# CraigIDent/SpliSER

Measured on AMD Instinct MI355X. Metric: splice sites/sec (+ reads/sec) processed, higher is better.
Workload: dtype int32/u32 counters, f64 SSE

## Files before the change

spliser_amd/csrc/spl_capi.cpp:

```cpp
#include <hip/hip_runtime_api.h>
#include <hip/hip_vector_types.h>

#include <sys/mman.h>

#include <algorithm>
#include <atomic>
#include <unistd.h>
#include <cstdarg>
#include <cstdio>
#include <cstring>
#include <new>
#include <string>
#include <chrono>
#include <condition_variable>
#include <functional>
#include <memory>
#include <mutex>
#include <thread>
#include <vector>

#include "../../include/spliser.h"
#include "spl_bam.h"
#include "spl_inflate.h"
#include "spl_sort.h"
// ... 208 lines not shown
}

extern "C" int spl_prof_enable(int on)
{
    std::lock_guard<std::mutex> lock(splprof::mu());
    for (const splprof::Rec &r : splprof::recs()) { splprof::pool().push_back({r.device, r.a}); splprof::pool().push_back({r.device, r.b}); }
    splprof::recs().clear();
    splprof::g_on.store(on ? 1 : 0);
    return SPL_OK;
}

extern "C" int spl_prof_report(char *buf, int cap)
{
    std::vector<splprof::Rec> recs;
    { std::lock_guard<std::mutex> lock(splprof::mu()); recs = splprof::recs(); }
    int cur = 0;
    const bool have = hipGetDevice(&cur) == hipSuccess;
    struct Sum { std::string name; int calls; double ms, bytes; };
    std::vector<Sum> sums;
    for (const splprof::Rec &r : recs) {
        (void)hipSetDevice(r.device);
        float ms = 0;
        if (hipEventSynchronize(r.b) != hipSuccess || hipEventElapsedTime(&ms, r.a, r.b) != hipSuccess) { (void)hipGetLastError(); continue; }
        size_t k = 0;
        while (k < sums.size() && sums[k].name != r.name) ++k;
        if (k == sums.size()) sums.push_back(Sum{r.name, 0, 0, 0});
        sums[k].calls++; sums[k].ms += ms; sums[k].bytes += r.bytes;
    }
    if (have) (void)hipSetDevice(cur);
    std::sort(sums.begin(), sums.end(), [](const Sum &a, const Sum &b) { return a.ms > b.ms; });
    std::string out = "[";
    for (size_t k = 0; k < sums.size(); ++k) {
        char line[256];
        snprintf(line, sizeof line, "%s{\"kernel\": \"%s\", \"calls\": %d, \"ms\": %.4f, \"bytes\": %.0f}", k ? ", " : "", sums[k].name.c_str(), sums[k].calls, sums[k].ms, sums[k].bytes);
        out += line;
    }
    out += "]";
    if (buf && cap > 0) { strncpy(buf, out.c_str(), (size_t)cap - 1); buf[cap - 1] = 0; }
    return (int)out.size() + 1;
}

struct spl_ctx {
    int device = -1;
    hipStream_t stream = nullptr;
    bool own_stream = false;
    hipEvent_t ev0 = nullptr, ev1 = nullptr;
    hipStream_t tail = nullptr;
    hipEvent_t ev_range[4] = {nullptr, nullptr, nullptr, nullptr}, ev_tail[4] = {nullptr, nullptr, nullptr, nullptr};
    uint64_t n_pass = 0;
    bool tail_pending = false;
    int32_t *d_err = nullptr;
    struct Stage { char *host = nullptr; size_t bytes = 0; hipEvent_t done = nullptr; bool busy = false, locked = false; };
    size_t stage_mb = 32;
    std::vector<Stage> stage;
    size_t stage_next = 0;
    hipStream_t copy = nullptr;
    hipEvent_t ev_copy = nullptr;
    int pack_threads = 1;
    bool stage_timing = false;
    hipEvent_t ev_t0 = nullptr, ev_t1 = nullptr;
    double tm_plan_s = 0, tm_emit_s = 0, tm_copy_ms = 0;
    size_t tm_bytes = 0, tm_pieces = 0;
    int last_grid = 0, last_lds = 0;
    struct Junction { int32_t left, right; uint8_t strand; uint32_t count, anchor_left, anchor_right; };
    std::vector<Junction> junctions;
    float junction_ms = -1.0f;
    int64_t junction_table_bytes = 0;
    std::vector<hipEvent_t> k_ev;
    int k_used = 0;
    bool k_on = false;
    std::vector<hipEvent_t> l_ev;
    int l_used = 0;
};

struct spl_dsites {
    int64_t n_sites = 0, n_part = 0, n_comp = 0;
    char *slab = nullptr;
    size_t slab_bytes = 0;
    int32_t *pos = nullptr;
    uint8_t *strand = nullptr, *flags = nullptr;
    uint4 *meta = nullptr;
    uint32_t *part_off = nullptr;
    int32_t *part_pos = nullptr, *part_site = nullptr, *comp_pos = nullptr;
    int64_t *alpha = nullptr, *edge_cnt = nullptr;
    uint32_t *bucket = nullptr;
    uint32_t n_buckets = 0;
    int32_t bucket_base = 0, bucket_shift = 0;
    bool has_sse_inputs = false;
    int32_t *diff = nullptr;
    int32_t *block_sums = nullptr;
    int32_t diff_stride = 0, scan_blocks = 0;
    int32_t n_dpos = 0;
    int32_t *dpos_first_row = nullptr;
    spl_dbk *dbucket = nullptr;
    uint32_t n_dbuckets = 0;
    int32_t dbase = 0;
    int32_t *flag_pos = nullptr;
    uint4 *jhash = nullptr;
    uint32_t jhash_mask = 0;
    uint4 *jrivals = nullptr;
    uint32_t *beta1 = nullptr, *beta2s = nullptr, *dbl = nullptr;
    size_t counter_bytes = 0;
    uint32_t *queue_n = nullptr;
    int32_t *err = nullptr;
    char *region[3] = {nullptr, nullptr, nullptr};
    size_t off_b2 = 0, off_dbl = 0, off_diff = 0, off_ctl = 0;
    bool region_clean[3] = {false, false, false};
    int cur = 2;
    void point_at(int k)
    {
        cur = k;
        beta1 = (uint32_t *)region[k]; beta2s = (uint32_t *)(region[k] + off_b2); dbl = (uint32_t *)(region[k] + off_dbl);
        diff = (int32_t *)(region[k] + off_diff); queue_n = (uint32_t *)(region[k] + off_ctl);
        err = (int32_t *)(region[k] + off_ctl + 4 * 8 * SPL_COUNTER_STRIDE);
    }
    int64_t *b2_simple = nullptr, *b2_cryptic = nullptr;
    double *b2_weighted = nullptr, *sse = nullptr;
    double *sse_cryptic = nullptr;
    bool sse_fused = false;
    const double *sse_view = nullptr;
};

struct DeviceReads;
struct spl_dreads {
    struct Segment {
        char *slab = nullptr;
        uint64_t rec_bytes = 0, n_wide = 0;
        int64_t n_reads = 0, n_ops = 0;
        int32_t shift = 0;
        std::vector<splpack::ChunkDesc> chunks;
        int group = -1;
        size_t group_seg = 0;
    };
    struct Group {
        DeviceReads *src = nullptr;
        std::vector<spl_layout_seg> segs;
        uint32_t n_chunks = 0;
        char *slab = nullptr;
        spl_layout_seg *d_segs = nullptr;
        spl_layout_chunk *d_chunks = nullptr;
    };
    std::vector<Segment> segs;
    std::vector<Group> groups;
    int64_t n_reads = 0, n_cigar = 0;
    uint32_t n_chunks = 0;
    uint32_t n_slots = 0;
    uint32_t chunk_shift = SPL_CHUNK_SHIFT;
    bool fused = false;
    bool finished = false;
    char *ctl = nullptr;
    spl_chunk_meta *meta = nullptr;
    uint32_t *cost = nullptr;
    uint32_t *chunk_order = nullptr;
    uint32_t *queue = nullptr;
    uint32_t *queue_alt = nullptr;
    uint32_t *queue_total = nullptr;
    uint32_t queue_cap = 0;
    mutable int queue_turn = 0;
    mutable bool queued_pass = false;
    mutable int64_t tail_pass = -1;
};

static inline size_t align_up(size_t v, size_t a = 256) { return (v + a - 1) / a * a; }

extern "C" int spl_device_count(int *n_out)
{
    if (!n_out) return spl_set_error(SPL_ERR_ARG, "spl_device_count: null output");
    int n = 0;
    hipError_t e = hipGetDeviceCount(&n);
    if (e != hipSuccess) { *n_out = 0; return spl_set_error(SPL_ERR_NO_DEVICE, "hipGetDeviceCount: %s", hipGetErrorString(e)); }
    *n_out = n;
    return SPL_OK;
}

static int create_ctx(int device_id, void *stream, bool use_given, spl_ctx **out)
{
    if (!out) return spl_set_error(SPL_ERR_ARG, "spl_create: null output");
    *out = nullptr;
    int n = 0;
    hipError_t e = hipGetDeviceCount(&n);
    if (e != hipSuccess || n <= 0)
        return spl_set_error(SPL_ERR_NO_DEVICE, "no HIP device visible (%s); libspliser_hip has no CPU fallback",
                             e == hipSuccess ? "device count 0" : hipGetErrorString(e));
    if (device_id < 0 || device_id >= n) return spl_set_error(SPL_ERR_ARG, "device %d out of range (0..%d)", device_id, n - 1);
    hipDeviceProp_t prop;
    HIP_TRY(hipGetDeviceProperties(&prop, device_id));
    if (strncmp(prop.gcnArchName, "gfx950", 6) != 0)
        return spl_set_error(SPL_ERR_NO_DEVICE, "device %d is %s; this library carries gfx950 (MI355X) code only", device_id,
                             prop.gcnArchName);
    HIP_TRY(hipSetDevice(device_id));
    spl_ctx *c = new (std::nothrow) spl_ctx();
    if (!c) return spl_set_error(SPL_ERR_NOMEM, "out of host memory");
    c->device = device_id;
    if (use_given) { c->stream = (hipStream_t)stream; c->own_stream = false; }
    else {
        hipError_t se = hipStreamCreateWithFlags(&c->stream, hipStreamNonBlocking);
        if (se != hipSuccess) { delete c; return spl_set_error(SPL_ERR_HIP, "hipStreamCreate: %s", hipGetErrorString(se)); }
        c->own_stream = true;
    }
    {
        const char *want_tail = getenv("SPL_TAIL_STREAM");
        if (!(want_tail && want_tail[0] == '0')) {
            bool ok = hipStreamCreateWithFlags(&c->tail, hipStreamNonBlocking) == hipSuccess;
            for (int i = 0; i < 4 && ok; ++i)
                ok = hipEventCreate(&c->ev_range[i]) == hipSuccess &&
                     hipEventCreateWithFlags(&c->ev_tail[i], hipEventDisableTiming | hipEventDisableSystemFence) == hipSuccess;
            if (!ok) {
                if (c->tail) (void)hipStreamDestroy(c->tail);
                c->tail = nullptr;
            }
        }
    }
    if (hipEventCreate(&c->ev0) != hipSuccess || hipEventCreate(&c->ev1) != hipSuccess ||
        hipMalloc((void **)&c->d_err, 16) != hipSuccess) {
        spl_destroy(c);
        return spl_set_error(SPL_ERR_HIP, "context resources could not be created");
    }
    *out = c;
    return SPL_OK;
}

extern "C" int spl_create(int device_id, spl_ctx **out) { return create_ctx(device_id, nullptr, false, out); }
extern "C" int spl_create_on_stream(int device_id, void *hip_stream, spl_ctx **out) { return create_ctx(device_id, hip_stream, true, out); }

static void free_stage(spl_ctx *c);

extern "C" void spl_destroy(spl_ctx *c)
{
    if (!c) return;
    (void)hipSetDevice(c->device);
    if (c->tail) (void)hipStreamSynchronize(c->tail);
    if (c->stream) (void)hipStreamSynchronize(c->stream);
    for (int i = 0; i < 4; ++i) {
        if (c->ev_range[i]) (void)hipEventDestroy(c->ev_range[i]);
        if (c->ev_tail[i]) (void)hipEventDestroy(c->ev_tail[i]);
    }
    if (c->tail) (void)hipStreamDestroy(c->tail);
    if (c->ev0) (void)hipEventDestroy(c->ev0);
    if (c->ev1) (void)hipEventDestroy(c->ev1);
    for (hipEvent_t e : c->k_ev) (void)hipEventDestroy(e);
    for (hipEvent_t e : c->l_ev) (void)hipEventDestroy(e);
    if (c->d_err) (void)hipFree(c->d_err);
    free_stage(c);
    if (c->own_stream && c->stream) (void)hipStreamDestroy(c->stream);
    delete c;
}

static hipError_t join_tail(spl_ctx *c)
{
    if (!c->tail || !c->tail_pending) return hipSuccess;
    c->tail_pending = false;
    return hipStreamWaitEvent(c->stream, c->ev_tail[(c->n_pass - 1) % 4], 0);
}

extern "C" int spl_sync(spl_ctx *c)
{
    if (!c) return spl_set_error(SPL_ERR_ARG, "spl_sync: null context");
    HIP_TRY(hipSetDevice(c->device));
    HIP_TRY(join_tail(c));
    HIP_TRY(hipStreamSynchronize(c->stream));
    return SPL_OK;
}

extern "C" int spl_pass_barrier(spl_ctx *c)
{
    if (!c) return spl_set_error(SPL_ERR_ARG, "spl_pass_barrier: null context");
    HIP_TRY(hipSetDevice(c->device));
    HIP_TRY(join_tail(c));
    return SPL_OK;
}

extern "C" int spl_timer_begin(spl_ctx *c)
{
    if (!c) return spl_set_error(SPL_ERR_ARG, "spl_timer_begin: null context");
    HIP_TRY(hipSetDevice(c->device));
    HIP_TRY(hipEventRecord(c->ev0, c->stream));
    return SPL_OK;
}

extern "C" int spl_timer_end(spl_ctx *c, float *ms)
{
    if (!c || !ms) return spl_set_error(SPL_ERR_ARG, "spl_timer_end: null argument");
    HIP_TRY(hipSetDevice(c->device));
    HIP_TRY(join_tail(c));
    HIP_TRY(hipEventRecord(c->ev1, c->stream));
    HIP_TRY(hipEventSynchronize(c->ev1));
    HIP_TRY(hipEventElapsedTime(ms, c->ev0, c->ev1));
    return SPL_OK;
}

extern "C" int spl_kernel_timing_begin(spl_ctx *c, int max_records)
{
    if (!c || max_records < 0) return spl_set_error(SPL_ERR_ARG, "spl_kernel_timing_begin: bad argument");
    HIP_TRY(hipSetDevice(c->device));
    while ((int)c->k_ev.size() < 2 * max_records) {
        hipEvent_t e;
        HIP_TRY(hipEventCreate(&e));
        c->k_ev.push_back(e);
    }
    while ((int)c->l_ev.size() < 2 * max_records) {
        hipEvent_t e;
        HIP_TRY(hipEventCreate(&e));
        c->l_ev.push_back(e);
    }
    c->k_used = 0;
    c->l_used = 0;
// ... 1855 lines not shown
        HIP_TRY(hipStreamSynchronize(st.k));
        if (counts.first_bad != none) {
            bad_line = header_lines + n_lines_all + (counts.first_bad >> 8) + 1;
            bad_reason = (uint32_t)(counts.first_bad & 0xffu);
            return STOPPED;
        }
        if (n_rec + kept_w > 0xfffffff0ull || n_ops + ops_w > 0xfffffff0ull) {
            bad_line = header_lines + n_lines_all + n_lines;
            bad_reason = SPL_SAM_TOO_MANY;
            return STOPPED;
        }
        n_drop_flags += counts.n_drop_flags;
        n_drop_mapq += counts.n_drop_mapq;
        if (want_stat) HIP_TRY((hipError_t)spl_dev_launch_bam_flagstat_reduce(d_fstat.as<uint32_t>(), (n_lines + 63u) / 64u, d_fsum.as<unsigned long long>(), st.k));
        { const int rc = make_room(kept_w, ops_w, win.hi - win.lo, fsize - win.hi); if (rc) return rc; }
        HIP_TRY((hipError_t)spl_dev_launch_sam_extract(text, base, d_lines.as<uint32_t>(), n_lines, last_end, &dev_names, opts.filter.min_mapq, opts.filter.require_flags,
                                                       opts.filter.exclude_flags, d_kept.as<uint32_t>(), d_nops.as<uint32_t>(), d_ltid.as<int32_t>(), n_rec, n_ops, cap_rec, cap_ops,
                                                       d_pos.as<int32_t>(), d_flag.as<uint16_t>(), d_tid.as<int32_t>(), d_cigoff.as<uint32_t>(), d_cigar.as<uint32_t>(),
                                                       want_xs ? d_xs.as<uint8_t>() : nullptr, d_maxend.as<unsigned long long>(), d_counts.as<spl_sam_counts>(), st.k));
        HIP_TRY((hipError_t)spl_dev_launch_sam_order(d_tid.as<int32_t>(), d_pos.as<int32_t>(), n_rec, kept_w, d_counts.as<spl_sam_counts>(), st.k));
        HIP_TRY(hipStreamSynchronize(st.k));
        n_rec += kept_w;
        n_ops += ops_w;
        n_lines_all += n_lines;
        {
            std::lock_guard<std::mutex> lock(mu);
            n_parsed = w + 1;
        }
        cv.notify_all();
        return SPL_OK;
    }

    void release_buffers()
    {
        for (DevBuf &b : d_text) b.release();
        d_chunks.release(); d_lines.release(); d_kept.release(); d_nops.release(); d_ltid.release(); d_fstat.release(); d_work.release();
    }
    std::vector<unsigned long long> maxend;
    int sort_records()
    {
        unsigned long long top = 1;
        for (unsigned long long e : maxend) top = std::max(top, e);
        sorter.plan(top, n_ref);
        release_buffers();
        const int rc = sorter.run(st.k, n_rec, n_ops, want_xs, d_pos, d_flag, d_cigoff, d_cigar, d_tid, d_xs);
        if (rc == SPL_OK) n_sorted = n_rec;
        return rc;
    }

    int finish()
    {
        if (!cap_rec) { const int rc = make_room(0, 0, 1, 0); if (rc) return rc; }
        const size_t nr = (size_t)std::max(n_ref, 1);
        const uint32_t bounds_cap = (uint32_t)nr + 1u;
        maxend.assign(nr, 0);
        spl_sam_counts counts;
        unsigned long long fsum[2 * SPL_FS_CATEGORIES] = {0};
        HIP_TRY(hipMemcpyAsync(maxend.data(), d_maxend.p, 8 * nr, hipMemcpyDeviceToHost, st.k));
        HIP_TRY(hipMemcpyAsync(&counts, d_counts.p, sizeof(counts), hipMemcpyDeviceToHost, st.k));
        if (want_stat) HIP_TRY(hipMemcpyAsync(fsum, d_fsum.p, sizeof(fsum), hipMemcpyDeviceToHost, st.k));
        HIP_TRY(hipStreamSynchronize(st.k));
        if (counts.overflow) return spl_set_error(SPL_ERR_HIP, "the SAM extraction disagreed with its scan (%u)", counts.overflow);
        if (counts.unordered) { const int rc = sort_records(); if (rc) return rc; }
        std::vector<uint64_t> bounds(2 * (size_t)bounds_cap, 0);
        uint32_t n_bounds = 0;
        HIP_TRY((hipError_t)spl_dev_launch_bam_bounds(d_tid.as<int32_t>(), d_cigoff.as<uint32_t>(), n_rec, d_bounds.as<uint64_t>(), d_nbounds.as<uint32_t>(), bounds_cap, st.k));
        HIP_TRY(hipMemcpyAsync(bounds.data(), d_bounds.p, 16 * (size_t)bounds_cap, hipMemcpyDeviceToHost, st.k));
        HIP_TRY(hipMemcpyAsync(&n_bounds, d_nbounds.p, 4, hipMemcpyDeviceToHost, st.k));
        HIP_TRY(hipStreamSynchronize(st.k));
        if (n_bounds > bounds_cap) return spl_set_error(SPL_ERR_HIP, "the SAM records' reference ids do not go up behind the sort");
        struct Run { uint64_t first; int32_t tid; uint32_t op; };
        std::vector<Run> runs;
        for (uint32_t k = 0; k < n_bounds; ++k) runs.push_back(Run{bounds[2 * k], (int32_t)(uint32_t)bounds[2 * k + 1], (uint32_t)(bounds[2 * k + 1] >> 32)});
        std::sort(runs.begin(), runs.end(), [](const Run &a, const Run &b) { return a.first < b.first; });
        for (size_t k = 0; k < runs.size(); ++k)
            if (runs[k].tid < 0 || runs[k].tid >= n_ref || (k && runs[k].tid <= runs[k - 1].tid)) return spl_set_error(SPL_ERR_HIP, "the SAM records' reference ids do not go up behind the sort");
        DeviceReads *keep = new (std::nothrow) DeviceReads();
        if (!keep) return spl_set_error(SPL_ERR_NOMEM, "out of host memory");
        keep->device = c->device;
        keep->n_rec = (int64_t)n_rec; keep->n_ops = (int64_t)n_ops;
        keep->ref_first.assign(nr, 0); keep->ref_n.assign(nr, 0); keep->ref_max.assign(nr, 0); keep->ref_ops.assign(nr, 0);
        for (size_t k = 0; k < runs.size(); ++k) {
            const size_t t = (size_t)runs[k].tid;
            const bool last = k + 1 == runs.size();
            keep->ref_first[t] = (int64_t)runs[k].first;
            keep->ref_n[t] = (int64_t)((last ? n_rec : runs[k + 1].first) - runs[k].first);
            keep->ref_ops[t] = (int64_t)((last ? n_ops : (uint64_t)runs[k + 1].op) - runs[k].op);
            keep->ref_max[t] = (int64_t)maxend[t];
        }
        keep->pos = d_pos.p; keep->flag = d_flag.p; keep->cig_off = d_cigoff.p; keep->cigar = d_cigar.p; keep->xs = d_xs.p;
        d_pos.p = d_flag.p = d_cigoff.p = d_cigar.p = d_xs.p = nullptr;
        res.reads = keep;
        res.totals.n_records = (int64_t)n_lines_all;
        res.totals.n_sorted = (int64_t)n_sorted;
        res.totals.sorted_on_device = n_sorted ? 1 : 0;
        res.totals.dropped[0] = (int64_t)n_drop_flags;
        res.totals.dropped[1] = (int64_t)n_drop_mapq;
        for (int q = 0; q < 2 * SPL_FS_CATEGORIES; ++q) res.totals.fstat[q] = (int64_t)fsum[q];
        if (timing)
            fprintf(stderr, "[spl_bam_decode_device] device %d: SAM text, %.1f MB in %zu window%s, %llu lines, %llu placed records%s: %.4f s\n", c->device, (fsize - begin) / 1e6, windows.size(),
                    windows.size() == 1 ? "" : "s", (unsigned long long)n_lines_all, (unsigned long long)n_rec, n_sorted ? ", sorted" : "", host_now() - t_begin);
        return SPL_OK;
    }
};
}

static int decode_text(spl_ctx *c, spl_bam *bam, ShareOut &res, const Publish &publish)
{
    HIP_TRY(hipSetDevice(c->device));
    SamDecode d(c, bam, res);
    int rc = d.plan();
    if (rc == SPL_OK) rc = d.set_up();
    for (size_t w = 0; w < d.windows.size() && rc == SPL_OK; ++w) rc = d.parse_window(w);
    if (rc == STOPPED) { spl_sam_fail(bam, d.bad_line, d.bad_reason); return SPL_OK; }
    if (rc == SPL_OK && d.long_line) { spl_sam_fail(bam, d.header_lines + d.n_lines_all + 1, SPL_SAM_LONG_LINE); return SPL_OK; }
    if (rc == SPL_OK) rc = d.finish();
    if (rc != SPL_OK) return rc;
    d.release_buffers();
    d.sorter.release();
    return publish(res);
}

extern "C" int spl_sort_keys_device(spl_ctx *c, const uint64_t *keys, int64_t n, int key_bits, uint32_t *perm_out)
{
    if (!c || n < 0 || (n && (!keys || !perm_out))) return spl_set_error(SPL_ERR_ARG, "spl_sort_keys_device: null argument");
    if (key_bits < 1 || key_bits > 64) return spl_set_error(SPL_ERR_ARG, "spl_sort_keys_device: key_bits %d is not in 1..64", key_bits);
    if ((uint64_t)n > 0xfffffff0ull) return spl_set_error(SPL_ERR_ARG, "spl_sort_keys_device: more than 2^32 keys");
    if (n == 0) return SPL_OK;
    HIP_TRY(hipSetDevice(c->device));
    uint32_t shifts[8];
    const uint32_t n_pass = spl_dev_sort_passes((uint32_t)std::min(key_bits, 32), (uint32_t)std::max(key_bits - 32, 0), shifts);
    DevBuf d_keys[2], d_perm[2], d_work;
    for (int k = 0; k < 2; ++k) { HIP_TRY(d_keys[k].get(8 * (size_t)n, c->stream)); HIP_TRY(d_perm[k].get(4 * (size_t)n, c->stream)); }
    HIP_TRY(d_work.get(spl_dev_sort_work_bytes((uint64_t)n), c->stream));
    HIP_TRY(hipMemcpyAsync(d_keys[0].p, keys, 8 * (size_t)n, hipMemcpyHostToDevice, c->stream));
    int cur = 0;
    for (uint32_t k = 0; k < n_pass; ++k, cur ^= 1)
        HIP_TRY((hipError_t)spl_dev_launch_sort_pass(d_keys[cur].as<uint64_t>(), k ? d_perm[cur].as<uint32_t>() : nullptr, (uint64_t)n, shifts[k], d_keys[cur ^ 1].as<uint64_t>(),
                                                     d_perm[cur ^ 1].as<uint32_t>(), d_work.p, c->stream));
    HIP_TRY(hipMemcpyAsync(perm_out, d_perm[cur].p, 4 * (size_t)n, hipMemcpyDeviceToHost, c->stream));
    HIP_TRY(hipStreamSynchronize(c->stream));
    return SPL_OK;
}

static int launch_layout(spl_ctx *c, spl_dreads *d)
{
    const uint32_t chunk = 1u << d->chunk_shift;
    std::vector<spl_layout_params> lps;
    for (spl_dreads::Group &g : d->groups) {
        spl_layout_params lp;
        lp.src = spl_devreads{(const int32_t *)g.src->pos, (const uint16_t *)g.src->flag, (const uint32_t *)g.src->cig_off, (const uint32_t *)g.src->cigar};
        lp.n_rec = g.src->n_rec; lp.n_ops = g.src->n_ops;
        lp.chunks = g.d_chunks; lp.rec_base = (uint8_t *)g.slab; lp.meta = d->meta;
        const int rc0 = spl_dev_launch_layout_map(&lp.src, g.d_segs, (uint32_t)g.segs.size(), g.n_chunks, chunk, g.d_chunks, d->cost, c->stream);
        if (rc0) return spl_set_error(SPL_ERR_HIP, "layout map kernel launch: %s", hipGetErrorString((hipError_t)rc0));
        lps.push_back(lp);
    }
    if (d->n_chunks) {
        splprof::Scope prof("spl_chunk_order_kernel", c->stream, 8.0 * (double)d->n_chunks);
        const int rc = spl_dev_launch_chunk_order(d->cost, d->n_chunks, chunk, d->chunk_order, c->stream);
        if (rc) return spl_set_error(SPL_ERR_HIP, "chunk order kernel launch: %s", hipGetErrorString((hipError_t)rc));
    }
    size_t gi = 0;
    if (d->fused) return SPL_OK;
    for (spl_dreads::Group &g : d->groups) {
        const spl_layout_params &lp = lps[gi++];
        int64_t n_reads = 0, n_ops = 0;
        for (const spl_layout_seg &ls : g.segs) n_reads += ls.n_reads;
        for (const spl_dreads::Segment &seg : d->segs) if (seg.group >= 0 && &d->groups[(size_t)seg.group] == &g) n_ops += seg.n_ops;
        const bool timed = c->k_on && (size_t)(2 * c->l_used + 1) < c->l_ev.size();
        int rc;
        {
            splprof::Scope prof("spl_layout_kernel", c->stream, 10.0 * (double)n_reads + 4.0 * (double)n_ops);
            rc = spl_dev_launch_layout(&lp, g.n_chunks, chunk, c->stream, timed ? (void *)c->l_ev[2 * c->l_used] : nullptr, timed ? (void *)c->l_ev[2 * c->l_used + 1] : nullptr);
        }
        if (timed) c->l_used++;
        if (rc) return spl_set_error(SPL_ERR_HIP, "layout kernel launch: %s", hipGetErrorString((hipError_t)rc));
    }
    return SPL_OK;
}

static bool fused_wanted()
{
    const char *e = getenv("SPL_FUSED");
    return !e || atoi(e) != 0;
}

static int finish_reads(spl_ctx *c, spl_dreads *d)
{
    if (d->finished) return SPL_OK;
    if (c->stage_timing && c->tm_pieces) {
        fprintf(stderr, "[spl_reads] %lld reads: classify %.4f s, write records %.4f s (host, %d threads); H2D %zu pieces, %.1f MB, %.3f ms in the copies = %.1f GB/s\n",
                (long long)d->n_reads, c->tm_plan_s, c->tm_emit_s, c->pack_threads, c->tm_pieces, c->tm_bytes / 1e6, c->tm_copy_ms,
                c->tm_copy_ms > 0 ? c->tm_bytes / 1e6 / c->tm_copy_ms : 0.0);
        c->tm_plan_s = c->tm_emit_s = c->tm_copy_ms = 0;
        c->tm_bytes = c->tm_pieces = 0;
    }
    if (d->n_cigar > 0xfffffff0LL) return spl_set_error(SPL_ERR_ARG, "more than 2^32 CIGAR ops in one read set: use more shards");
    auto host_now = []() { return std::chrono::duration<double>(std::chrono::steady_clock::now().time_since_epoch()).count(); };
    const double tf0 = host_now();
    bool all_device = !d->segs.empty();
    for (const spl_dreads::Segment &seg : d->segs) all_device = all_device && seg.group >= 0;
    d->fused = fused_wanted() && all_device && d->groups.size() == 1;
    const size_t n = d->n_chunks;
    const uint32_t per = spl_order_per((uint32_t)n);
    d->n_slots = 8u * per;
    const size_t shard_cap = (size_t)per << d->chunk_shift;
    size_t off = 0;
    auto take = [&](size_t bytes) { size_t o = off; off = align_up(off + bytes); return o; };
    const size_t o_meta = take(sizeof(spl_chunk_meta) * std::max<size_t>(n, 1)), o_cost = take(4 * std::max<size_t>(n, 1)), o_order = take(4 * std::max<size_t>(d->n_slots, 1));
    const size_t o_total = take(4);
    const size_t o_queue = take(4 * 8 * shard_cap), o_queue_alt = take(c->tail ? 4 * 8 * shard_cap : 0);
    hipError_t e = devmem::get((void **)&d->ctl, std::max<size_t>(off, 256), 'c');
    if (e != hipSuccess) return spl_set_error(SPL_ERR_HIP, "hipMalloc(%zu) for the read set: %s", off, hipGetErrorString(e));
    d->meta = (spl_chunk_meta *)(d->ctl + o_meta);
    d->cost = (uint32_t *)(d->ctl + o_cost);
    d->chunk_order = (uint32_t *)(d->ctl + o_order);
    d->queue_total = (uint32_t *)(d->ctl + o_total);
    d->queue = (uint32_t *)(d->ctl + o_queue);
    d->queue_alt = c->tail ? (uint32_t *)(d->ctl + o_queue_alt) : d->queue;
    d->queue_cap = (uint32_t)shard_cap;
    const double tf_alloc = host_now() - tf0;
    hipError_t q = hipSuccess;
    std::vector<spl_chunk_meta> meta;
    std::vector<uint32_t> cost;
    bool host_segs = false;
    {
        size_t k = 0;
        for (const spl_dreads::Segment &seg : d->segs) {
            if (seg.group >= 0) { k += d->groups[(size_t)seg.group].segs[seg.group_seg].n_chunks; continue; }
            if (seg.chunks.empty()) continue;
            if (!host_segs) { meta.resize(n); cost.resize(n); host_segs = true; }
            const uint64_t rec_al = align_up((size_t)seg.rec_bytes);
            const size_t k0 = k;
            for (const splpack::ChunkDesc &cd : seg.chunks) {
                spl_chunk_meta &m = meta[k];
                m.rec = (uint64_t)(uintptr_t)seg.slab + cd.rec_off;
                m.wide = (uint64_t)(uintptr_t)seg.slab + rec_al;
                m.shift = seg.shift;
                m.first_pos = cd.first_pos;
                for (int r = 0; r < SPL_RC_RUNS; ++r) m.n[r] = cd.n[r];
                cost[k++] = cd.cost;
            }
            if (c->copy == nullptr) { int rc = ensure_stage(c); if (rc) return rc; }
            if (q == hipSuccess) q = hipMemcpyAsync(d->meta + k0, meta.data() + k0, sizeof(spl_chunk_meta) * (k - k0), hipMemcpyHostToDevice, c->copy);
            if (q == hipSuccess) q = hipMemcpyAsync(d->cost + k0, cost.data() + k0, 4 * (k - k0), hipMemcpyHostToDevice, c->copy);
        }
    }
    if (q == hipSuccess && c->copy && (host_segs || !c->stage.empty())) q = hipStreamSynchronize(c->copy);
    for (spl_ctx::Stage &st : c->stage) st.busy = false;
    if (q != hipSuccess) return spl_set_error(SPL_ERR_HIP, "read set upload: %s", hipGetErrorString(q));
    const uint32_t chunk = 1u << d->chunk_shift;
    for (spl_dreads::Group &g : d->groups) {
        const size_t seg_bytes = align_up(sizeof(spl_layout_seg) * g.segs.size());
        e = d->fused ? hipSuccess : devmem::get((void **)&g.slab, SPL_LAYOUT_SLOT(chunk) * (size_t)g.n_chunks + 256, 'R');
        if (e == hipSuccess) e = devmem::get((void **)&g.d_segs, seg_bytes + sizeof(spl_layout_chunk) * (size_t)g.n_chunks + 16, 'd');
        if (e != hipSuccess) return spl_set_error(SPL_ERR_HIP, "hipMalloc for the device layout of %u chunks: %s", g.n_chunks, hipGetErrorString(e));
        g.d_chunks = (spl_layout_chunk *)((char *)g.d_segs + seg_bytes);
        HIP_TRY(hipMemcpyAsync(g.d_segs, g.segs.data(), sizeof(spl_layout_seg) * g.segs.size(), hipMemcpyHostToDevice, c->stream));
    }
    const int rc = launch_layout(c, d);
    if (rc) return rc;
    if (c->stage_timing)
        fprintf(stderr, "[spl_reads_finish] %zu chunks (%zu group(s) laid out on the device): control block (%.1f MB) at %.4f s, launched %.4f\n", n, d->groups.size(), off / 1e6,
                tf_alloc, host_now() - tf0);
    d->finished = true;
    return SPL_OK;
}

static int unfuse(spl_ctx *c, spl_dreads *d)
{
    if (!d->fused) return SPL_OK;
    const uint32_t chunk = 1u << d->chunk_shift;
    int rc = SPL_OK;
    for (spl_dreads::Group &g : d->groups) {
        const hipError_t e = devmem::get((void **)&g.slab, SPL_LAYOUT_SLOT(chunk) * (size_t)g.n_chunks + 256, 'R');
        if (e != hipSuccess) { rc = spl_set_error(SPL_ERR_HIP, "hipMalloc for the device layout of %u chunks: %s", g.n_chunks, hipGetErrorString(e)); break; }
    }
    if (rc == SPL_OK) {
        d->fused = false;
        rc = launch_layout(c, d);
    }
    if (rc != SPL_OK) {
        d->fused = true;
        for (spl_dreads::Group &g : d->groups)
            if (g.slab) { devmem::put(g.slab); g.slab = nullptr; }
    }
    return rc;
}

extern "C" int spl_reads_relayout(spl_ctx *c, spl_dreads *d)
{
    if (!c || !d) return spl_set_error(SPL_ERR_ARG, "spl_reads_relayout: null argument");
    if (!d->finished) return spl_set_error(SPL_ERR_ARG, "spl_reads_relayout: the read set is not finished (spl_reads_finish)");
    if (d->groups.empty()) return spl_set_error(SPL_ERR_ARG, "spl_reads_relayout: no segment of this read set was laid out on the device");
    HIP_TRY(hipSetDevice(c->device));
    if (c->tail && d->tail_pass >= 0 && (uint64_t)d->tail_pass + 3 > c->n_pass) HIP_TRY(hipStreamWaitEvent(c->stream, c->ev_tail[d->tail_pass % 4], 0));
    return launch_layout(c, d);
}

static int source_of(const spl_reads *r, splpack::Source &src, int64_t *max_end, const char *who)
{
    if (r->n_reads < 0) return spl_set_error(SPL_ERR_ARG, "%s: negative n_reads", who);
    if (r->n_reads && (!r->pos || !r->flag || !r->cig_off)) return spl_set_error(SPL_ERR_ARG, "read set has null arrays");
    if (r->n_reads && r->cig_off[0] != 0) return spl_set_error(SPL_ERR_ARG, "cig_off[0] must be 0");
    const int64_t g = r->n_reads ? r->cig_off[r->n_reads] : 0;
    if (g && !r->cigar) return spl_set_error(SPL_ERR_ARG, "cigar is null");
    if (r->n_reads) src.add(splpack::Part{r->pos, r->flag, r->cig_off, r->cigar, r->n_reads});
    *max_end = -1;
    return SPL_OK;
}

extern "C" int spl_pack_host(const spl_reads *reads, int n_threads, int64_t *n_chunks_out, int64_t *rec_bytes_out, int64_t *n_wide_out,
                             void *chunk_desc, void *rec, uint32_t *wide)
{
    if (!reads || !n_chunks_out || !rec_bytes_out || !n_wide_out) return spl_set_error(SPL_ERR_ARG, "spl_pack_host: null argument");
    splpack::Source src;
    int64_t max_end;
    int rc = source_of(reads, src, &max_end, "spl_pack_host");
    if (rc) return rc;
    splpack::Plan plan;
    splpack::plan(src, plan, n_threads > 0 ? n_threads : 1);
    *n_chunks_out = (int64_t)plan.chunks.size();
    *rec_bytes_out = (int64_t)plan.rec_bytes;
    *n_wide_out = (int64_t)plan.n_wide;
    static_assert(sizeof(splpack::ChunkDesc) == 32, "chunk descriptors are handed out as 32-byte records");
    if (chunk_desc && !plan.chunks.empty()) memcpy(chunk_desc, plan.chunks.data(), sizeof(splpack::ChunkDesc) * plan.chunks.size());
    if (rec && !plan.chunks.empty()) {
        std::vector<uint32_t> no_wide((size_t)plan.n_wide + 1);
        memset(rec, 0, (size_t)plan.rec_bytes);
        splpack::emit(src, plan, 0, plan.chunks.size(), (uint8_t *)rec, wide ? wide : no_wide.data());
    }
    return SPL_OK;
}

extern "C" int spl_reads_begin_sized(spl_ctx *c, int64_t expected_reads, spl_dreads **out)
{
    if (!c || !out) return spl_set_error(SPL_ERR_ARG, "spl_reads_begin: null argument");
    *out = new (std::nothrow) spl_dreads();
    if (!*out) return spl_set_error(SPL_ERR_NOMEM, "out of host memory");
    bool big = expected_reads >= SPL_BIG_SET_READS;
    if (const char *e = getenv("SPL_FORCE_CHUNK")) big = atol(e) == SPL_CHUNK_BIG;
    (*out)->chunk_shift = big ? SPL_CHUNK_BIG_SHIFT : SPL_CHUNK_SHIFT;
    return SPL_OK;
}

extern "C" int spl_reads_begin(spl_ctx *c, spl_dreads **out) { return spl_reads_begin_sized(c, 0, out); }

static int64_t max_end_of(const spl_reads *r)
{
    int64_t best = 0;
    for (int64_t i = 0; i < r->n_reads; ++i) {
        int64_t len = 0;
        for (uint32_t k = r->cig_off[i]; k < r->cig_off[i + 1]; ++k) {
            const uint32_t code = r->cigar[k] & 15u;
            if (code == 0 || code == 2 || code == 3 || code == 7 || code == 8) len += r->cigar[k] >> 4;
        }
        const int64_t e = (int64_t)r->pos[i] + (len > 0 ? len : 1) - 1;
        if (e > best && e <= (int64_t)SPL_COORD_MAX) best = e;
    }
    return best;
}

extern "C" int spl_reads_add(spl_ctx *c, spl_dreads *d, const spl_reads *reads, int32_t pos_shift) { return spl_reads_add2(c, d, reads, pos_shift, -1); }

extern "C" int spl_reads_add2(spl_ctx *c, spl_dreads *d, const spl_reads *reads, int32_t pos_shift, int64_t known_max_end)
{
    if (!c || !d || !reads) return spl_set_error(SPL_ERR_ARG, "spl_reads_add: null argument");
    HIP_TRY(hipSetDevice(c->device));
    splpack::Source src;
// ... 175 lines not shown
    if (!h) { free_device_reads(dev); return spl_set_error(SPL_ERR_NOMEM, "out of host memory"); }
    h->reads = dev;
    *out = h;
    return SPL_OK;
}

extern "C" void spl_soa_free(spl_ctx *c, spl_dsoa *soa)
{
    if (!soa) return;
    if (c) (void)hipSetDevice(c->device);
    free_device_reads(soa->reads);
    delete soa;
}

extern "C" int spl_reads_add_soa(spl_ctx *c, spl_dreads *d, spl_dsoa *soa, int seg, int32_t pos_shift)
{
    if (!c || !d || !soa) return spl_set_error(SPL_ERR_ARG, "spl_reads_add_soa: null argument");
    DeviceReads *dev = soa->reads;
    if (seg < 0 || (size_t)seg >= dev->ref_n.size()) return spl_set_error(SPL_ERR_ARG, "spl_reads_add_soa: no segment %d", seg);
    if (dev->device != c->device) return spl_set_error(SPL_ERR_ARG, "spl_reads_add_soa: the arrays are on device %d, the context on %d", dev->device, c->device);
    HIP_TRY(hipSetDevice(c->device));
    const size_t t = (size_t)seg;
    return add_segment_device(c, d, dev, dev->ref_first[t], dev->ref_n[t], dev->ref_ops[t], pos_shift, dev->ref_n[t] && pos_shift != 0 ? dev->ref_max[t] : -1);
}

extern "C" int spl_reads_has_strand(const spl_dreads *d, int *out)
{
    if (!d || !out) return spl_set_error(SPL_ERR_ARG, "spl_reads_has_strand: null argument");
    *out = d->finished && d->fused && d->groups.size() == 1 && d->groups[0].src->xs ? 1 : 0;
    return SPL_OK;
}

extern "C" int spl_reads_layout_bytes(spl_ctx *c, const spl_dreads *d, int64_t *soa_bytes_out, int64_t *record_bytes_out)
{
    if (!c || !d || !soa_bytes_out || !record_bytes_out) return spl_set_error(SPL_ERR_ARG, "spl_reads_layout_bytes: null argument");
    if (!d->finished) return spl_set_error(SPL_ERR_ARG, "spl_reads_layout_bytes: the read set is not finished (spl_reads_finish)");
    HIP_TRY(hipSetDevice(c->device));
    int64_t soa = 0, rec = 0;
    std::vector<spl_chunk_meta> meta(d->n_chunks);
    if (d->fused) {
        for (const spl_dreads::Segment &seg : d->segs) soa += 10 * seg.n_reads + 4 * seg.n_ops;
        *soa_bytes_out = soa;
        *record_bytes_out = 0;
        return SPL_OK;
    }
    if (d->n_chunks) {
        HIP_TRY(hipMemcpyAsync(meta.data(), d->meta, sizeof(spl_chunk_meta) * d->n_chunks, hipMemcpyDeviceToHost, c->stream));
        HIP_TRY(hipStreamSynchronize(c->stream));
    }
    size_t k = 0;
    for (const spl_dreads::Segment &seg : d->segs) {
        const size_t nc = seg.group >= 0 ? d->groups[(size_t)seg.group].segs[seg.group_seg].n_chunks : seg.chunks.size();
        if (seg.group >= 0) {
            soa += 10 * seg.n_reads + 4 * seg.n_ops;
            for (size_t j = 0; j < nc; ++j) rec += (int64_t)spl_run_offset(meta[k + j].n, 4);
        }
        k += nc;
    }
    *soa_bytes_out = soa;
    *record_bytes_out = rec;
    return SPL_OK;
}

extern "C" int spl_reads_finish(spl_ctx *c, spl_dreads *d)
{
    if (!c || !d) return spl_set_error(SPL_ERR_ARG, "spl_reads_finish: null argument");
    HIP_TRY(hipSetDevice(c->device));
    return finish_reads(c, d);
}

extern "C" void spl_reads_free(spl_ctx *c, spl_dreads *d)
{
    if (!d) return;
    if (c) (void)hipSetDevice(c->device);
    if (c && c->copy) (void)hipStreamSynchronize(c->copy);
    if (c && c->tail) (void)hipStreamSynchronize(c->tail);
    if (c && c->stream) (void)hipStreamSynchronize(c->stream);
    for (spl_dreads::Segment &seg : d->segs) devmem::put(seg.slab);
    for (spl_dreads::Group &g : d->groups) { devmem::put(g.slab); devmem::put(g.d_segs); free_device_reads(g.src); }
    devmem::put(d->ctl);
    delete d;
}

extern "C" int spl_reads_upload_segments(spl_ctx *c, int n_seg, const spl_reads *segs, const int32_t *pos_shift, spl_dreads **out)
{
    if (!c || !out || n_seg < 0 || (n_seg && (!segs || !pos_shift)))
        return spl_set_error(SPL_ERR_ARG, "spl_reads_upload_segments: null argument");
    *out = nullptr;
    spl_dreads *d = nullptr;
    int64_t total = 0;
    for (int k = 0; k < n_seg; ++k) total += segs[k].n_reads > 0 ? segs[k].n_reads : 0;
    int rc = spl_reads_begin_sized(c, total, &d);
    for (int k = 0; k < n_seg && rc == SPL_OK; ++k) rc = spl_reads_add(c, d, &segs[k], pos_shift[k]);
    if (rc == SPL_OK) rc = spl_reads_finish(c, d);
    if (rc != SPL_OK) { spl_reads_free(c, d); return rc; }
    *out = d;
    return SPL_OK;
}

extern "C" int spl_reads_upload(spl_ctx *c, const spl_reads *r, spl_dreads **out)
{
    if (!c || !r || !out) return spl_set_error(SPL_ERR_ARG, "spl_reads_upload: null argument");
    const int32_t zero = 0;
    return spl_reads_upload_segments(c, 1, r, &zero, out);
}

extern "C" int spl_count_launch(spl_ctx *c, spl_dsites *ds, const spl_dreads *dr, const spl_opts *o)
{
    if (!c || !ds || !dr || !o) return spl_set_error(SPL_ERR_ARG, "spl_count_launch: null argument");
    if (o->stranded < 0 || o->stranded > 2)
        return spl_set_error(SPL_ERR_ARG, "stranded must be 0 (unstranded), 1 (fr) or 2 (rf); the reference raises "
                                          "UnboundLocalError for any other strandedType");
    HIP_TRY(hipSetDevice(c->device));
    const bool pairs = (o->flags & SPL_OPT_PAIR_KERNEL) != 0;
    const bool piped = c->tail != nullptr && !pairs && ds->region_clean[(ds->cur + 1) % 3];
    if (piped) {
        if (c->n_pass >= 2) HIP_TRY(hipStreamWaitEvent(c->stream, c->ev_tail[(c->n_pass - 2) % 4], 0));
    } else
        HIP_TRY(join_tail(c));
    const int next = (ds->cur + 1) % 3;
    if (ds->region_clean[next]) {
        ds->point_at(next);
        ds->region_clean[next] = false;
    } else if (int rc0 = spl_dev_launch_clear(ds->beta1, ds->counter_bytes, c->stream))
        return spl_set_error(SPL_ERR_HIP, "clear kernel launch: %s", hipGetErrorString((hipError_t)rc0));
    if (!dr->finished) return spl_set_error(SPL_ERR_ARG, "spl_count_launch: the read set is not finished (spl_reads_finish)");
    if (dr->fused && pairs) { const int rc0 = unfuse(c, const_cast<spl_dreads *>(dr)); if (rc0) return rc0; }
    uint32_t *const queue = dr->queue_turn ? dr->queue_alt : dr->queue;
    dr->queue_turn ^= 1;
    dr->queued_pass = false;
    ds->sse_fused = false;
    spl_count_params p;
    memset(&p, 0, sizeof(p));
    p.n_reads = dr->n_reads;
    p.n_chunks = dr->n_chunks;
    p.chunk_meta = dr->meta;
    p.n_sites = (int32_t)ds->n_sites;
    p.site_pos = ds->pos; p.site_strand = ds->strand; p.site_flags = ds->flags; p.site_meta = ds->meta;
    p.part_pos = ds->part_pos; p.part_site = ds->part_site; p.comp_pos = ds->comp_pos;
    p.diff = ds->diff; p.diff_stride = ds->diff_stride;
    p.dbucket = ds->dbucket; p.n_dbuckets = ds->n_dbuckets; p.dbase = ds->dbase; p.n_dpos = ds->n_dpos;
    p.dpos_first_row = ds->dpos_first_row;
    p.jhash = ds->jhash; p.jhash_mask = ds->jhash_mask; p.jrivals = ds->jrivals;
    spl_hot_params h;
    memset(&h, 0, sizeof(h));
    h.n_chunks = dr->n_slots; h.chunk_shift = dr->chunk_shift; h.chunk_meta = dr->meta; h.chunk_order = dr->chunk_order; h.part_pos = ds->part_pos;
    h.dbucket = p.dbucket; h.n_dbuckets = p.n_dbuckets; h.dbase = p.dbase; h.n_dpos = p.n_dpos;
    h.stranded = o->stranded; h.diff = p.diff; h.diff_stride = p.diff_stride;
    h.queue = queue; h.queue_n = ds->queue_n; h.err = ds->err;
    h.queue_cap = dr->queue_cap;
    if (dr->fused) {
        const spl_dreads::Group &g = dr->groups[0];
        h.cells = g.d_chunks;
        h.src = spl_devreads{(const int32_t *)g.src->pos, (const uint16_t *)g.src->flag, (const uint32_t *)g.src->cig_off, (const uint32_t *)g.src->cigar};
        h.src_n_rec = g.src->n_rec; h.src_n_ops = g.src->n_ops;
    }
    h.jhash = ds->jhash; h.jhash_mask = ds->jhash_mask; h.jrivals = ds->jrivals; h.dbl = ds->dbl; h.combine_mode = o->combine_mode ? 1 : 0;

    p.bucket = ds->bucket; p.n_buckets = ds->n_buckets; p.bucket_base = ds->bucket_base; p.bucket_shift = ds->bucket_shift;
    p.stranded = o->stranded; p.combine_mode = o->combine_mode ? 1 : 0;
    p.beta1 = ds->beta1; p.beta2s_reads = ds->beta2s; p.dbl = ds->dbl; p.err = ds->err;
    int grid = 0, lds = 0;
    const bool timed = c->k_on && (size_t)(2 * c->k_used + 1) < c->k_ev.size();
    hipEvent_t ev_stop = timed ? c->k_ev[2 * c->k_used + 1] : (piped ? c->ev_range[c->n_pass % 4] : nullptr);
    int64_t alg = 0;
    if (splprof::g_on.load(std::memory_order_relaxed)) (void)spl_count_algorithmic_bytes(ds, dr, &alg);
    int rc;
    { splprof::Scope prof("spl_count_ranges_kernel", c->stream, (double)alg); rc = spl_dev_launch_count(&p, &h, pairs, c->stream, &grid, &lds, timed ? (void *)c->k_ev[2 * c->k_used] : nullptr, (void *)ev_stop); }
    if (timed) c->k_used++;
    c->last_grid = grid;
    c->last_lds = lds;
    if (rc != 0) return spl_set_error(SPL_ERR_HIP, "count kernel launch: %s", hipGetErrorString((hipError_t)rc));
    if (!pairs && grid > 0) {
        hipStream_t ts = c->stream;
        if (piped) {
            HIP_TRY(hipStreamWaitEvent(c->tail, ev_stop, 0));
            ts = c->tail;
        }
        const int to_clear = piped ? (ds->cur + 2) % 3 : (ds->cur + 1) % 3;
        spl_queue_params lq;
        lq.queue = queue; lq.queue_n = ds->queue_n; lq.queue_cap = h.queue_cap; lq.chunk_shift = dr->chunk_shift; lq.queue_total = dr->queue_total;
        lq.clear_region = (uint4 *)ds->region[to_clear]; lq.clear_n16 = ds->counter_bytes / 16;
        lq.cells = h.cells; lq.src = h.src;
        lq.diff = ds->diff; lq.block_sums = ds->block_sums; lq.diff_stride = ds->diff_stride; lq.n_dpos = ds->n_dpos;
        lq.scan_blocks = ds->scan_blocks; lq.scan_arrays = o->stranded ? 4 : 2;
        rc = spl_dev_launch_literal(&p, &lq, ts);
        if (rc != 0) return spl_set_error(SPL_ERR_HIP, "literal kernel launch: %s", hipGetErrorString((hipError_t)rc));
        ds->region_clean[to_clear] = true;
        dr->queued_pass = true;
        spl_scan_params q;
        memset(&q, 0, sizeof(q));
        q.n_dpos = ds->n_dpos; q.dpos_first_row = ds->dpos_first_row;
        q.n_arrays = o->stranded ? 4 : 2; q.diff_stride = ds->diff_stride;
        q.n_blocks = ds->scan_blocks; q.diff = ds->diff; q.block_sums = ds->block_sums; q.site_flags = ds->flags;
        q.beta1 = ds->beta1; q.beta2s_reads = ds->beta2s;
        q.with_sse = ds->has_sse_inputs ? 1 : 0;
        if (q.with_sse) {
            q.sse.n_sites = ds->n_sites; q.sse.site_pos = ds->pos; q.sse.part_off = ds->part_off; q.sse.part_pos = ds->part_pos;
            q.sse.part_site = ds->part_site; q.sse.alpha = ds->alpha; q.sse.edge_cnt = ds->edge_cnt; q.sse.dbl = ds->dbl;
            q.sse.beta2_simple = ds->b2_simple; q.sse.beta2_cryptic = ds->b2_cryptic; q.sse.beta2_weighted = ds->b2_weighted;
            q.sse.sse = ds->sse; q.sse_with_cryptic = ds->sse_cryptic;
        }
        rc = spl_dev_launch_scan(&q, ts);
        if (rc != 0) return spl_set_error(SPL_ERR_HIP, "scan kernel launch: %s", hipGetErrorString((hipError_t)rc));
        ds->sse_fused = q.with_sse != 0;
        if (piped) {
            HIP_TRY(hipEventRecord(c->ev_tail[c->n_pass % 4], c->tail));
            dr->tail_pass = (int64_t)c->n_pass;
            c->n_pass++;
            c->tail_pending = true;
        }
    }
    return SPL_OK;
}

extern "C" int spl_sse_launch(spl_ctx *c, spl_dsites *ds, int cryptic)
{
    if (!c || !ds) return spl_set_error(SPL_ERR_ARG, "spl_sse_launch: null argument");
    if (!ds->has_sse_inputs) return spl_set_error(SPL_ERR_ARG, "spl_sse needs sites->alpha, sites->edge_cnt and sites->part_site");
    HIP_TRY(hipSetDevice(c->device));
    if (ds->sse_fused) {
        ds->sse_view = cryptic ? ds->sse_cryptic : ds->sse;
        return SPL_OK;
    }
    ds->sse_view = ds->sse;
    HIP_TRY(join_tail(c));
    spl_sse_params p;
    memset(&p, 0, sizeof(p));
    p.n_sites = ds->n_sites; p.site_pos = ds->pos; p.part_off = ds->part_off; p.part_pos = ds->part_pos; p.part_site = ds->part_site;
    p.alpha = ds->alpha; p.edge_cnt = ds->edge_cnt; p.beta1 = ds->beta1; p.beta2s_reads = ds->beta2s; p.dbl = ds->dbl;
    p.cryptic = cryptic ? 1 : 0;
    p.beta2_simple = ds->b2_simple; p.beta2_cryptic = ds->b2_cryptic; p.beta2_weighted = ds->b2_weighted; p.sse = ds->sse;
    int rc = spl_dev_launch_sse(&p, c->stream);
    if (rc != 0) return spl_set_error(SPL_ERR_HIP, "spl_sse_kernel launch: %s", hipGetErrorString((hipError_t)rc));
    return SPL_OK;
}

static int check_device_error(spl_ctx *c, const spl_dsites *ds)
{
    int32_t err = 0;
    HIP_TRY(join_tail(c));
    HIP_TRY(hipMemcpyAsync(&err, ds->err, sizeof(err), hipMemcpyDeviceToHost, c->stream));
    HIP_TRY(hipStreamSynchronize(c->stream));
    if (err & SPL_DEV_ERR_TABLE) return spl_set_error(SPL_ERR_HIP, "a wave's list of reads overflowed in the range kernel (internal error: results discarded)");
    if (err & SPL_DEV_ERR_RANGE)
        return spl_set_error(SPL_ERR_RANGE, "a read starts below 0 or ends beyond coordinate %d: split the shard (spliser_amd/shard.py)", SPL_COORD_MAX);
    return SPL_OK;
}

extern "C" int spl_counters_download(spl_ctx *c, const spl_dsites *ds, uint32_t *beta1, uint32_t *b2s, uint32_t *dbl)
{
    if (!c || !ds) return spl_set_error(SPL_ERR_ARG, "spl_counters_download: null argument");
    HIP_TRY(hipSetDevice(c->device));
    HIP_TRY(join_tail(c));
    if (beta1 && ds->n_sites) HIP_TRY(hipMemcpyAsync(beta1, ds->beta1, 4 * ds->n_sites, hipMemcpyDeviceToHost, c->stream));
    if (b2s && ds->n_sites) HIP_TRY(hipMemcpyAsync(b2s, ds->beta2s, 4 * ds->n_sites, hipMemcpyDeviceToHost, c->stream));
    if (dbl && ds->n_part) HIP_TRY(hipMemcpyAsync(dbl, ds->dbl, 4 * ds->n_part, hipMemcpyDeviceToHost, c->stream));
    return check_device_error(c, ds);
}

extern "C" int spl_sse_download(spl_ctx *c, const spl_dsites *ds, int64_t *b2s, int64_t *b2c, double *b2w, double *sse)
{
    if (!c || !ds) return spl_set_error(SPL_ERR_ARG, "spl_sse_download: null argument");
    HIP_TRY(hipSetDevice(c->device));
    const size_t n = 8 * (size_t)ds->n_sites;
    HIP_TRY(join_tail(c));
    if (n) {
        if (b2s) HIP_TRY(hipMemcpyAsync(b2s, ds->b2_simple, n, hipMemcpyDeviceToHost, c->stream));
        if (b2c) HIP_TRY(hipMemcpyAsync(b2c, ds->b2_cryptic, n, hipMemcpyDeviceToHost, c->stream));
        if (b2w) HIP_TRY(hipMemcpyAsync(b2w, ds->b2_weighted, n, hipMemcpyDeviceToHost, c->stream));
        if (sse) HIP_TRY(hipMemcpyAsync(sse, ds->sse_view, n, hipMemcpyDeviceToHost, c->stream));
    }
    HIP_TRY(hipStreamSynchronize(c->stream));
    return SPL_OK;
}

extern "C" int spl_count_algorithmic_bytes(const spl_dsites *ds, const spl_dreads *dr, int64_t *out)
{
    if (!ds || !dr || !out) return spl_set_error(SPL_ERR_ARG, "spl_count_algorithmic_bytes: null argument");
    const int64_t R = dr->n_reads, G = dr->n_cigar, S = ds->n_sites, P = ds->n_part, C = ds->n_comp;
    *out = R * (4 + 2 + 4) + 4 * G + S * (4 + 1 + 8) + 4 * (P + C) + S * 8 + 4 * P;
    return SPL_OK;
}

extern "C" int spl_junctions(spl_ctx *c, const spl_dreads *dr, int stranded, int32_t min_anchor, int32_t min_intron, int32_t max_intron,
                             int64_t *n_out)
{
    if (!c || !dr || !n_out) return spl_set_error(SPL_ERR_ARG, "spl_junctions: null argument");
    if (min_anchor < 0 || min_intron < 0 || max_intron < 0) return spl_set_error(SPL_ERR_ARG, "spl_junctions: negative filter value");
    if (stranded < 0 || stranded > 3) return spl_set_error(SPL_ERR_ARG, "stranded must be 0, 1 (fr), 2 (rf) or 3 (the reads' strand bytes)");
    HIP_TRY(hipSetDevice(c->device));
    c->junctions.clear();
    *n_out = 0;
    if (!dr->finished) return spl_set_error(SPL_ERR_ARG, "spl_junctions: the read set is not finished (spl_reads_finish)");
    const bool fused = dr->fused && dr->groups.size() == 1;
    const spl_dreads::Group *g = fused ? &dr->groups[0] : nullptr;
    if (stranded == 3 && !fused)
        return spl_set_error(SPL_ERR_ARG, "spl_junctions: stranded = 3 needs a fused read set (all of it from one device decode or one spl_soa_upload3)");
    if (stranded == 3 && !g->src->xs)
        return spl_set_error(SPL_ERR_ARG, "spl_junctions: stranded = 3, but the reads have no strand bytes (spl_bam_set_aux_strand before the decode, or spl_soa_upload3)");
    spl_devreads src{nullptr, nullptr, nullptr, nullptr};
    uint64_t wanted = (uint64_t)dr->n_cigar;
    hipEvent_t ev0 = nullptr, ev1 = nullptr;
    c->junction_ms = -1.0f;
    if (fused) {
        src = spl_devreads{(const int32_t *)g->src->pos, (const uint16_t *)g->src->flag, (const uint32_t *)g->src->cig_off, (const uint32_t *)g->src->cigar};
// ... 235 lines not shown
```

spliser_amd/csrc/spl_device.h:

```cpp
#ifndef SPL_DEVICE_H
#define SPL_DEVICE_H

#include <stdint.h>
#include <hip/hip_vector_types.h>

#include "spl_pack.h"
#include "spl_devpack.h"

#ifndef SPL_BLOCK
#define SPL_BLOCK 256
#endif
#define SPL_COUNTER_STRIDE 64
#define SPL_WAVES (SPL_BLOCK / 64)
#ifndef SPL_K_SIMPLE
#define SPL_K_SIMPLE 4
#define SPL_K_MNM 2
#endif
#ifndef SPL_LIST_K
#define SPL_LIST_K 2
#endif
#ifndef SPL_WAVE_ITERS
#define SPL_WAVE_ITERS 10
#endif
#define SPL_WAVE_READS (64 * SPL_WAVE_ITERS)
#define SPL_TILE_FUSED_SHIFT 10
#define SPL_TILE_FUSED (1 << SPL_TILE_FUSED_SHIFT)
#define SPL_BLOCK_FUSED 256
#define SPL_WAVE_READS_FUSED 512
#define SPL_REC_BYTES_FUSED 16448
#define SPL_WIN 1020
#define SPL_WIN_STRANDED 956
#define SPL_WIN_STRANDED_FUSED 508
#define SPL_SERIAL_MAX 8
#ifndef SPL_AGG_ROUNDS
#define SPL_AGG_ROUNDS 2
#endif
#define SPL_LITERAL_WAVES 8192
#ifndef SPL_SCAN_BLOCK
#define SPL_SCAN_BLOCK 256
#endif


#define SPL_DEV_ERR_RANGE 1
#define SPL_DEV_ERR_TABLE 2

#define SPL_JF_COUNT_MASK 0x00ffffffu
#define SPL_JF_COMPLEX 0x40000000u
#define SPL_JF_MULTIROW 0x80000000u

#define SPL_SF_PLUS 1u
#define SPL_SF_MINUS 2u

struct spl_dbk {
    uint32_t first;
    uint32_t occ;
    uint32_t rival;
};

struct spl_count_params {
    int64_t n_reads;
    uint32_t n_chunks;
    const spl_chunk_meta *chunk_meta;
    int32_t n_sites;
    const int32_t *site_pos;
    const uint8_t *site_strand;
    const uint8_t *site_flags;
    const uint4 *site_meta;
    const int32_t *part_pos;
    const int32_t *part_site;
    const int32_t *comp_pos;
    const uint32_t *bucket;
    uint32_t n_buckets;
    int32_t bucket_base;
    int32_t bucket_shift;
    const spl_dbk *dbucket;
    uint32_t n_dbuckets;
    int32_t dbase;
    int32_t n_dpos;
    const int32_t *dpos_first_row;
    const uint4 *jhash;
    uint32_t jhash_mask;
    const uint4 *jrivals;
    int32_t stranded;
    int32_t combine_mode;
    uint32_t *beta1;
    uint32_t *beta2s_reads;
    uint32_t *dbl;
    int32_t *diff;
    int32_t diff_stride;
    int32_t *err;
};

struct spl_hot_params {
    uint32_t n_chunks;
    uint32_t chunk_shift;
    const spl_chunk_meta *chunk_meta;
    const uint32_t *chunk_order;
    const int32_t *part_pos;
    const spl_dbk *dbucket;
    uint32_t n_dbuckets;
    int32_t dbase;
    int32_t n_dpos;
    int32_t stranded;
    int32_t *diff;
    int32_t diff_stride;
    const uint4 *jhash;
    uint32_t jhash_mask;
    const uint4 *jrivals;
    uint32_t *dbl;
    int32_t combine_mode;
    uint32_t *queue;
    uint32_t *queue_n;
    uint32_t queue_cap;
    int32_t *err;
    const spl_layout_chunk *cells;
    spl_devreads src;
    int64_t src_n_rec, src_n_ops;
};

struct spl_queue_params {
    const uint32_t *queue;
    const uint32_t *queue_n;
    uint32_t queue_cap;
    uint32_t chunk_shift;
    uint32_t *queue_total;
    const int32_t *diff;
    int32_t *block_sums;
    int32_t diff_stride, n_dpos, scan_blocks, scan_arrays;
    uint4 *clear_region;
    size_t clear_n16;
    const spl_layout_chunk *cells;
    spl_devreads src;
};

struct spl_sse_params {
    int64_t n_sites;
    const int32_t *site_pos;
    const uint32_t *part_off;
    const int32_t *part_pos;
    const int32_t *part_site;
    const int64_t *alpha;
    const int64_t *edge_cnt;
    const uint32_t *beta1;
    const uint32_t *beta2s_reads;
    const uint32_t *dbl;
    int32_t cryptic;
    int64_t *beta2_simple;
    int64_t *beta2_cryptic;
    double *beta2_weighted;
    double *sse;
};

struct spl_scan_params {
    int32_t n_dpos;
    const int32_t *dpos_first_row;
    int32_t n_arrays;
    int32_t diff_stride;
    int32_t n_blocks;
    const int32_t *diff;
    int32_t *block_sums;
    const uint8_t *site_flags;
    uint32_t *beta1;
    uint32_t *beta2s_reads;
    int32_t with_sse;
    spl_sse_params sse;
    double *sse_with_cryptic;
};


#ifdef __cplusplus
extern "C" {
#endif
int spl_dev_launch_count(const spl_count_params *p, const spl_hot_params *h, int pairs, void *stream, int *grid_out, int *lds_out, void *ev_start, void *ev_stop);
int spl_dev_launch_junctions(const spl_chunk_meta *chunk_meta, uint32_t n_chunks,
                             int stranded, uint32_t min_anchor, uint32_t min_intron, uint32_t max_intron, unsigned long long *keys,
                             uint32_t *vals, uint32_t n_slots, unsigned long long *out_keys,
                             uint32_t *out_vals, uint32_t *n_out, int32_t *err, void *stream);
int spl_dev_launch_build_dbuckets(const int32_t *site_pos, const int32_t *dpos_first_row, int32_t n_dpos, const int32_t *flag_pos,
                                  int32_t n_flag, int32_t dbase, uint32_t n_dbuckets, spl_dbk *out, void *stream);
int spl_dev_launch_clear(void *region, size_t bytes, void *stream);
int spl_dev_launch_literal(const spl_count_params *p, const spl_queue_params *q, void *stream);
int spl_dev_launch_scan(const spl_scan_params *p, void *stream);
int spl_dev_launch_sse(const spl_sse_params *p, void *stream);
#ifdef __cplusplus
}
#endif

#endif
```

spliser_amd/csrc/spl_devpack.h:

```cpp
#ifndef SPL_DEVPACK_H
#define SPL_DEVPACK_H
#include <stdint.h>

#include "spl_pack.h"

struct spl_devreads {
    const int32_t *pos;
    const uint16_t *flag;
    const uint32_t *cig_off;
    const uint32_t *cigar;
};

struct spl_layout_seg {
    int64_t first;
    int64_t n_reads;
    uint32_t chunk0;
    uint32_t dev0;
    uint32_t n_chunks;
    int32_t shift;
};

#define SPL_LAYOUT_SLOT(chunk_reads) ((size_t)(chunk_reads) * SPL_REC_OTHER + 256u)

struct spl_layout_chunk {
    int64_t lo;
    uint32_t n;
    uint32_t o_lo, o_hi;
    uint32_t seg_op0;
    int32_t shift;
    uint32_t flat;
};

struct spl_layout_params {
    spl_devreads src;
    int64_t n_rec;
    int64_t n_ops;
    const spl_layout_chunk *chunks;
    uint8_t *rec_base;
    spl_chunk_meta *meta;
};

static inline uint32_t spl_layout_seg_chunks(int64_t first, int64_t n_reads, uint32_t chunk)
{
    return n_reads > 0 ? (uint32_t)((first + n_reads - 1) / chunk - first / chunk + 1) : 0u;
}
static inline uint32_t spl_order_per(uint32_t n_chunks) { return ((n_chunks + 7u) / 8u + 7u) / 8u * 8u; }

#ifdef __cplusplus
extern "C" {
#endif
int spl_dev_launch_layout_map(const spl_devreads *src, const spl_layout_seg *segs, uint32_t n_segs, uint32_t n_chunks, uint32_t chunk, spl_layout_chunk *chunks, uint32_t *cost,
                              void *stream);
int spl_dev_launch_layout(const spl_layout_params *p, uint32_t n_dev_chunks, uint32_t chunk, void *stream, void *ev_start, void *ev_stop);
int spl_dev_launch_chunk_order(const uint32_t *cost, uint32_t n_chunks, uint32_t chunk, uint32_t *order, void *stream);
#ifdef __cplusplus
}
#endif
#endif
```

spliser_amd/csrc/spl_devpack.hip:

```cpp
#include <hip/hip_runtime.h>
#include <hip/hip_ext.h>
#include <stdint.h>

#include "spl_pack.h"
#include "spl_devpack.h"
#include "spl_layout_tile.h"

using namespace spllay;

__global__ __launch_bounds__(256) void spl_layout_map_kernel(const spl_devreads src, const spl_layout_seg *segs, uint32_t n_segs, uint32_t n_chunks, uint32_t chunk,
                                                             spl_layout_chunk *chunks, uint32_t *cost)
{
    const uint32_t k = blockIdx.x * 256u + threadIdx.x;
    if (k >= n_chunks) return;
    uint32_t a = 0, b = n_segs;
    while (b - a > 1u) {
        const uint32_t mid = (a + b) >> 1;
        if (segs[mid].dev0 <= k) a = mid; else b = mid;
    }
    const spl_layout_seg s = segs[a];
    const int64_t cell = s.first / chunk + (int64_t)(k - s.dev0), c0 = cell * (int64_t)chunk, c1 = c0 + chunk;
    spl_layout_chunk c;
    c.lo = s.first > c0 ? s.first : c0;
    const int64_t hi = s.first + s.n_reads < c1 ? s.first + s.n_reads : c1;
    c.n = (uint32_t)(hi - c.lo);
    c.o_lo = src.cig_off[c.lo]; c.o_hi = src.cig_off[hi]; c.seg_op0 = src.cig_off[s.first];
    c.shift = s.shift;
    c.flat = s.chunk0 + (k - s.dev0);
    chunks[k] = c;
    cost[c.flat] = (3u * (c.o_hi - c.o_lo) + c.n) / 2u;
}

template <int C>
__global__ __launch_bounds__(C / 4) __attribute__((amdgpu_waves_per_eu(8, 8))) void spl_layout_kernel(const spl_layout_params p)
{
    constexpr uint32_t T = C / 4, NW = T / 64, STAGE = 4 * C;
    __shared__ uint32_t s_ops[STAGE];
    __shared__ uint32_t s_cnt[NW][2];
    __shared__ int32_t s_first;
    const uint32_t k = blockIdx.x;
    const spl_layout_chunk ch = p.chunks[k];
    uint32_t n[4];
    layout_tile<C>(p.src, p.n_rec, p.n_ops, ch, (lay_lds_w32 *)s_ops, (lay_lds_w32 *)&s_cnt[0][0], (lay_lds_i32 *)&s_first, RecordsInMemory{p.rec_base, SPL_LAYOUT_SLOT(C)}, n);
    if (threadIdx.x == 0) {
        uint8_t *const rec = p.rec_base + (size_t)k * SPL_LAYOUT_SLOT(C);
        spl_chunk_meta m;
        m.rec = (uint64_t)(uintptr_t)rec;
        m.wide = (uint64_t)(uintptr_t)(p.src.cigar + ch.seg_op0);
        m.shift = ch.shift;
        m.first_pos = s_first;
        m.n[0] = (uint16_t)n[0]; m.n[1] = (uint16_t)n[1]; m.n[2] = (uint16_t)n[2]; m.n[3] = (uint16_t)n[3];
        p.meta[ch.flat] = m;
    }
}

__global__ __launch_bounds__(1024) void spl_chunk_order_kernel(const uint32_t *cost, uint32_t n, uint32_t per, uint32_t *order)
{
    constexpr uint32_t NB = 4096;
    __shared__ uint32_t s_hist[NB];
    __shared__ uint32_t s_part[1024];
    const uint32_t x = blockIdx.x, t = threadIdx.x;
    for (uint32_t b = t; b < NB; b += 1024u) s_hist[b] = 0;
    __syncthreads();
    auto chunk_of = [&](uint32_t e) { return (x + 8u * (e >> 3)) * 8u + (e & 7u); };
    auto key_of = [&](uint32_t c) { const uint32_t q = c >> 4; return NB - 1u - (q < NB ? q : NB - 1u); };
    for (uint32_t e = t; e < per; e += 1024u) {
        const uint32_t j = chunk_of(e);
        if (j < n) atomicAdd(&s_hist[key_of(cost[j])], 1u);
    }
    __syncthreads();
    const uint32_t h0 = s_hist[4 * t], h1 = s_hist[4 * t + 1], h2 = s_hist[4 * t + 2], h3 = s_hist[4 * t + 3];
    s_part[t] = h0 + h1 + h2 + h3;
    __syncthreads();
    for (uint32_t s = 1; s < 1024u; s <<= 1) {
        const uint32_t a = t >= s ? s_part[t - s] : 0u;
        __syncthreads();
        s_part[t] += a;
        __syncthreads();
    }
    const uint32_t before = s_part[t] - (h0 + h1 + h2 + h3), total = s_part[1023];
    __syncthreads();
    s_hist[4 * t] = before; s_hist[4 * t + 1] = before + h0; s_hist[4 * t + 2] = before + h0 + h1; s_hist[4 * t + 3] = before + h0 + h1 + h2;
    __syncthreads();
    uint32_t *const mine = order + (size_t)x * per;
    for (uint32_t e = t; e < per; e += 1024u) {
        const uint32_t j = chunk_of(e);
        if (j < n) mine[atomicAdd(&s_hist[key_of(cost[j])], 1u)] = j;
    }
    for (uint32_t s = total + t; s < per; s += 1024u) mine[s] = 0xffffffffu;
}

extern "C" int spl_dev_launch_layout_map(const spl_devreads *src, const spl_layout_seg *segs, uint32_t n_segs, uint32_t n_chunks, uint32_t chunk, spl_layout_chunk *chunks,
                                         uint32_t *cost, void *stream)
{
    if (!n_segs || !n_chunks) return 0;
    hipLaunchKernelGGL(spl_layout_map_kernel, dim3((n_chunks + 255u) / 256u), dim3(256), 0, (hipStream_t)stream, *src, segs, n_segs, n_chunks, chunk, chunks, cost);
    return (int)hipGetLastError();
}

extern "C" int spl_dev_launch_layout(const spl_layout_params *p, uint32_t n_dev_chunks, uint32_t chunk, void *stream, void *ev_start, void *ev_stop)
{
    if (!n_dev_chunks) return 0;
    hipStream_t st = (hipStream_t)stream;
    hipEvent_t e0 = (hipEvent_t)ev_start, e1 = (hipEvent_t)ev_stop;
    if (chunk == (uint32_t)SPL_CHUNK) hipExtLaunchKernelGGL(spl_layout_kernel<SPL_CHUNK>, dim3(n_dev_chunks), dim3(SPL_CHUNK / 4), 0, st, e0, e1, 0, *p);
    else if (chunk == (uint32_t)SPL_CHUNK_BIG) hipExtLaunchKernelGGL(spl_layout_kernel<SPL_CHUNK_BIG>, dim3(n_dev_chunks), dim3(SPL_CHUNK_BIG / 4), 0, st, e0, e1, 0, *p);
    else return (int)hipErrorInvalidValue;
    return (int)hipGetLastError();
}

extern "C" int spl_dev_launch_chunk_order(const uint32_t *cost, uint32_t n_chunks, uint32_t chunk, uint32_t *order, void *stream)
{
    if (!n_chunks) return 0;
    (void)chunk;
    hipLaunchKernelGGL(spl_chunk_order_kernel, dim3(8), dim3(1024), 0, (hipStream_t)stream, cost, n_chunks, spl_order_per(n_chunks), order);
    return (int)hipGetLastError();
}
```

spliser_amd/csrc/spl_kernels.hip:

```cpp
#include <hip/hip_runtime.h>
#include <hip/hip_ext.h>
#include <cstdio>
#include <cstdlib>
#include <stdint.h>

#define SPL_HD __device__ __forceinline__
#include "spl_classify.h"
#include "spl_device.h"
#include "spl_layout_tile.h"

namespace {

__device__ __forceinline__ int32_t first_site_at_or_after(const spl_count_params &p, int32_t pos)
{
    const int64_t rel = (int64_t)pos - (int64_t)p.bucket_base;
    uint32_t b = 0;
    if (rel > 0) {
        const int64_t q = rel >> p.bucket_shift;
        b = q >= (int64_t)p.n_buckets ? p.n_buckets : (uint32_t)q;
    }
    uint32_t lo = p.bucket[b];
    uint32_t hi = p.bucket[b < p.n_buckets ? b + 1 : b];
    while (lo < hi) {
        const uint32_t mid = (lo + hi) >> 1;
// ... 221 lines not shown
__device__ __forceinline__ bool jt_find(const uint4 *jhash, uint32_t jhash_mask, int32_t l, int32_t r, uint4 &ent)
{
    uint32_t h = (uint32_t)l * 0x9E3779B1u ^ (uint32_t)r * 0x85EBCA77u;
    h ^= h >> 15;
    for (int probe = 0; probe < 8; ++probe) {
        ent = jhash[2u * ((h + (uint32_t)probe) & jhash_mask)];
        if ((int32_t)ent.x == l && (int32_t)ent.y == r) return true;
        if (ent.x == 0x80000000u) return false;
    }
    return false;
}

template <bool STRANDED>
__device__ __forceinline__ void rivals_literal(const spl_count_params &p, int32_t pos, uint32_t flag, const uint32_t *ops,
                                               uint32_t n_ops, int32_t end_fetch)
{
    int32_t cur = pos;
    for (uint32_t k = 0; k < n_ops; ++k) {
        const uint32_t op = ops[k];
        const uint32_t code = op & 15u;
        if (!((SPL_PROG_MASK >> code) & 1u)) continue;
        const int32_t d = (int32_t)(op >> 4);
        cur += d;
        if (code != SPL_OP_N) continue;
        const int32_t l = cur - d - 1, r = cur - 1;
        uint4 ent;
        if (!jt_find(p.jhash, p.jhash_mask, l, r, ent)) continue;
        {
            bool repeat = false;
            int32_t c2 = pos;
            for (uint32_t k2 = 0; k2 < k; ++k2) {
                const uint32_t op2 = ops[k2];
                if (!((SPL_PROG_MASK >> (op2 & 15u)) & 1u)) continue;
                const int32_t d2 = (int32_t)(op2 >> 4);
                c2 += d2;
                repeat |= (op2 & 15u) == SPL_OP_N && c2 - d2 - 1 == l && c2 - 1 == r;
            }
            if (repeat) continue;
        }
        const uint32_t n_riv = ent.w & SPL_JF_COUNT_MASK;
        for (uint32_t i = 0; i < n_riv; ++i) {
            const uint4 rx = p.jrivals[2u * (ent.z + i) + 1u];
            const int32_t trow = (int32_t)rx.x;
            const int32_t t = p.site_pos[trow];
            if (t < pos || t > end_fetch) continue;
            bool earlier = false;
            int32_t c2 = pos;
            for (uint32_t k2 = 0; k2 < k && !earlier; ++k2) {
                const uint32_t op2 = ops[k2];
                if (!((SPL_PROG_MASK >> (op2 & 15u)) & 1u)) continue;
                const int32_t d2 = (int32_t)(op2 >> 4);
                c2 += d2;
                if ((op2 & 15u) != SPL_OP_N) continue;
                uint4 e2;
                if (!jt_find(p.jhash, p.jhash_mask, c2 - d2 - 1, c2 - 1, e2)) continue;
                for (uint32_t i2 = 0; i2 < (e2.w & SPL_JF_COUNT_MASK); ++i2) earlier |= p.jrivals[2u * (e2.z + i2) + 1u].x == rx.x;
            }
            if (earlier) continue;
            const uint4 mt = p.site_meta[trow];
            const int32_t *part = p.part_pos + mt.x;
            const int32_t *comp = p.comp_pos + mt.z;
            bool strand_ok = true;
            if (STRANDED) strand_ok = (p.site_strand[trow] == spl_read_strand(flag, p.stranded));
            const spl_pair full = spl_classify_pair(pos, ops, n_ops, t, part, mt.y, comp, mt.w, strand_ok);
            const spl_pair base = spl_classify_pair(pos, ops, n_ops, t, nullptr, 0u, nullptr, 0u, strand_ok);
            if (full.cls == base.cls) continue;
            if (base.cls == SPL_CLS_BETA1) agg_add(&p.beta1[trow], -1);
            else if (base.cls == SPL_CLS_ME) agg_add(&p.beta2s_reads[trow], -1);
            apply_pair_global(p, full, trow, pos, ops, n_ops, part, mt.y, mt.x);
        }
    }
}

template <bool STRANDED>
__device__ __forceinline__ void unmapped_read(const spl_count_params &p, int32_t pos, uint32_t flag, const uint32_t *ops, uint32_t n_ops)
{
    const int32_t n_sites = p.n_sites;
    for (int32_t s = first_site_at_or_after(p, pos); s < n_sites && p.site_pos[s] == pos; ++s) {
        bool strand_ok = true;
        if (STRANDED) strand_ok = (p.site_strand[s] == spl_read_strand(flag, p.stranded));
        const uint4 m = p.site_meta[s];
        const spl_pair r = spl_classify_pair(pos, ops, n_ops, pos, p.part_pos + m.x, m.y, p.comp_pos + m.z, m.w, strand_ok);
        apply_pair_global(p, r, s, pos, ops, n_ops, p.part_pos + m.x, m.y, m.x);
    }
}

template <class P>
__device__ __forceinline__ uint32_t dbk_slot(const P &p, int32_t x)
{
    int32_t b = (x - p.dbase) >> 5;
    b = b < 0 ? 0 : b;
    const int32_t last = (int32_t)p.n_dbuckets - 1;
    return (uint32_t)(b > last ? last : b);
}

template <class P>
__device__ __forceinline__ void dbk_resolve(const P &p, int32_t x, const spl_dbk &e, int32_t &u, uint32_t &nv)
{
    const uint32_t bit = (uint32_t)(x - p.dbase) & 31u;
    u = (int32_t)(e.first + (uint32_t)__popc(e.occ & ((1u << bit) - 1u)));
    nv = (e.occ >> bit) & 1u;
}

template <class P>
__device__ __forceinline__ void dbk_resolve(const P &p, int32_t x, const spl_dbk &e, int32_t &u, uint32_t &nv, uint32_t &rv)
{
    dbk_resolve(p, x, e, u, nv);
    rv = (e.rival >> ((uint32_t)(x - p.dbase) & 31u)) & 1u;
}

typedef __attribute__((address_space(3))) int32_t spl_lds_i32;

template <int NARR, int WIN = (NARR == 4 ? SPL_WIN_STRANDED : SPL_WIN)>
__device__ __forceinline__ void commit_key(const spl_hot_params &p, spl_lds_i32 *lds, int32_t wbase, bool valid, uint32_t key, int32_t sign)
{
    if (valid) {
        const int arr = (int)(key & 3u);
        const int32_t d = (int32_t)(key >> 2);
        const uint32_t loc = (uint32_t)(d - wbase);
        if (loc <= (uint32_t)WIN) __hip_atomic_fetch_add(lds + (arr * (WIN + 1) + (int)loc), sign, __ATOMIC_RELAXED, __HIP_MEMORY_SCOPE_WORKGROUP);
        else atomicAdd(&p.diff[(int64_t)arr * p.diff_stride + d], sign);
    }
}

template <int NARR, int WIN>
__device__ __forceinline__ void commit_range(const spl_hot_params &p, spl_lds_i32 *lds, int32_t wbase, bool em, int32_t lo, int32_t ub, uint32_t arr)
{
    const uint32_t a = (uint32_t)(lo - wbase), b = (uint32_t)(ub - wbase);
    const bool inside = a <= (uint32_t)WIN && b <= (uint32_t)WIN;
    if (em && inside) {
        spl_lds_i32 *const row = lds + (int)arr * (WIN + 1);
        __hip_atomic_fetch_add(row + (int)a, 1, __ATOMIC_RELAXED, __HIP_MEMORY_SCOPE_WORKGROUP);
        __hip_atomic_fetch_add(row + (int)b, -1, __ATOMIC_RELAXED, __HIP_MEMORY_SCOPE_WORKGROUP);
    }
    if (__any(em && !inside)) {
        commit_key<NARR, WIN>(p, lds, wbase, em && !inside, ((uint32_t)lo << 2) | arr, 1);
        commit_key<NARR, WIN>(p, lds, wbase, em && !inside, ((uint32_t)ub << 2) | arr, -1);
    }
}

__device__ __forceinline__ spl_dbk dbk_load2(const spl_hot_params &p, uint32_t s)
{
    typedef __attribute__((address_space(1))) const uint32_t gdw;
    gdw *q = (gdw *)((__attribute__((address_space(1))) const char *)p.dbucket + (size_t)((s << 3) + (s << 2)));
    spl_dbk e; e.first = q[0]; e.occ = q[1]; e.rival = 0u;
    return e;
}

template <bool STRANDED, int NARR, int WIN, int R>
struct SimpleInPlace {
    static constexpr bool in_place = true;
    const spl_hot_params &p;
    spl_lds_i32 *lds;
    int32_t wbase, shift;
    bool active;
    spl_dbk e0[R], e1[R];
    __device__ __forceinline__ void issue(int j, bool is_simple, uint32_t w0, uint32_t w1)
    {
        if (!active || !__any(is_simple)) return;
        const int32_t a = (int32_t)w0 + shift, b = a + (int32_t)(w1 >> 16);
        e0[j] = e1[j] = spl_dbk{0u, 0u, 0u};
        if (is_simple) {
            e0[j] = dbk_load2(p, dbk_slot(p, a - 1));
            e1[j] = dbk_load2(p, dbk_slot(p, b - 1));
        }
    }
    __device__ __forceinline__ void commit(int j, bool is_simple, uint32_t w0, uint32_t w1)
    {
        if (!active || !__any(is_simple)) return;
        const int32_t a = (int32_t)w0 + shift, b = a + (int32_t)(w1 >> 16);
        int32_t ua, ub; uint32_t nva, nvb;
        dbk_resolve(p, a - 1, e0[j], ua, nva);
        dbk_resolve(p, b - 1, e1[j], ub, nvb);
        const int32_t lo = ua + (int32_t)nva;
        const bool emit = is_simple && ub > lo;
        uint32_t arr = 0;
        if (STRANDED) arr = (spl_read_strand(w1 & 0xffffu, p.stranded) == (uint8_t)'-') ? 1u : 0u;
        if (__any(emit)) commit_range<NARR, WIN>(p, lds, wbase, emit, lo, ub, arr);
    }
};

__device__ __forceinline__ void agg_add(uint32_t *addr, int32_t delta)
{
    const int lane = (int)__builtin_amdgcn_mbcnt_hi(~0u, __builtin_amdgcn_mbcnt_lo(~0u, 0u));
    unsigned long long todo = __ballot(1);
    const uint32_t lo = (uint32_t)(uintptr_t)addr, hi = (uint32_t)((uintptr_t)addr >> 32);
    for (int round = 0; round < SPL_AGG_ROUNDS; ++round) {
        const int leader = __ffsll((long long)todo) - 1;
        const bool same = (__shfl((int)lo, leader) == (int)lo) && (__shfl((int)hi, leader) == (int)hi);
        const unsigned long long grp = __ballot(same);
        const unsigned long long plus = __ballot(same && delta > 0);
        if (lane == leader) {
            const int32_t sum = 2 * (int32_t)__popcll(plus) - (int32_t)__popcll(grp);
            if (sum) atomicAdd(addr, (uint32_t)sum);
        }
        if (same) return;
        todo &= ~grp;
    }
    atomicAdd(addr, (uint32_t)delta);
}


__device__ __forceinline__ uint32_t junction_hash(int32_t l, int32_t r)
{
    uint32_t h = (uint32_t)l * 0x9E3779B1u ^ (uint32_t)r * 0x85EBCA77u;
    return h ^ (h >> 15);
}

template <bool STRANDED, int NARR, int WIN = (NARR == 4 ? SPL_WIN_STRANDED : SPL_WIN)>
__device__ __forceinline__ bool rivals_inline_from(const spl_hot_params &p, spl_lds_i32 *lds, int32_t wbase, int32_t l, int32_t r, uint32_t h,
                                                   uint4 ent, uint4 first, const int32_t *blk_a, const int32_t *blk_b, uint32_t sidx)
{
    bool found = false;
    for (int probe = 0; probe < 8; ++probe) {
        if (probe) {
            const uint4 *slot = p.jhash + 2u * ((h + (uint32_t)probe) & p.jhash_mask);
            ent = slot[0];
            first = slot[1];
        }
        if ((int32_t)ent.x == l && (int32_t)ent.y == r) { found = true; break; }
        if (ent.x == 0x80000000u) break;
    }
    if (!found) return true;
    const uint32_t n_riv = ent.w & SPL_JF_COUNT_MASK;
    if ((ent.w & SPL_JF_COMPLEX) || n_riv > 4u) return false;
    if (!STRANDED && (ent.w & SPL_JF_MULTIROW)) return false;
    for (uint32_t i = 0; i < n_riv; ++i) {
        const uint4 rv = i ? p.jrivals[2u * (ent.z + i)] : first;
        const int32_t t = (int32_t)rv.x;
        const uint32_t td = rv.y & 0x3fffffffu;
        if (STRANDED && ((rv.y >> 30) != (sidx ? 2u : 1u))) continue;
        const uint32_t a_b1 = sidx, a_me = (STRANDED ? 2u : 1u) + sidx;
        if (t > l && t < r) {
            commit_key<NARR, WIN>(p, lds, wbase, true, (td << 2) | a_me, -1);
            commit_key<NARR, WIN>(p, lds, wbase, true, ((td + 1u) << 2) | a_me, 1);
        } else {
            bool cov = false;
#pragma unroll
            for (int j = 0; j < 2; ++j) cov |= (blk_a[j] <= t) && (t + 1 <= blk_b[j]);
            if (cov) {
                commit_key<NARR, WIN>(p, lds, wbase, true, (td << 2) | a_b1, -1);
                commit_key<NARR, WIN>(p, lds, wbase, true, ((td + 1u) << 2) | a_b1, 1);
                commit_key<NARR, WIN>(p, lds, wbase, true, (td << 2) | a_me, 1);
                commit_key<NARR, WIN>(p, lds, wbase, true, ((td + 1u) << 2) | a_me, -1);
                if (rv.z != 0xffffffffu) agg_add(&p.dbl[rv.z & 0x7fffffffu], 1);
                if (rv.w != 0xffffffffu) agg_add(&p.dbl[rv.w], 1);
            }
        }
    }
    return true;
}

template <bool STRANDED, int NARR, int WIN = (NARR == 4 ? SPL_WIN_STRANDED : SPL_WIN)>
__device__ __forceinline__ bool rivals_inline2(const spl_hot_params &p, spl_lds_i32 *lds, int32_t wbase, const int32_t (&jl)[2],
                                               const int32_t (&jr)[2], const bool (&flagged)[2], const int32_t (&blk_a)[3],
                                               const int32_t (&blk_b)[3], uint32_t sidx)
{
    uint32_t r_off[2] = {0, 0}, r_n[2] = {0, 0};
    uint4 ent[2], first[2];
    uint32_t h[2];
#pragma unroll
    for (int j = 0; j < 2; ++j) {
        h[j] = (uint32_t)jl[j] * 0x9E3779B1u ^ (uint32_t)jr[j] * 0x85EBCA77u;
        h[j] ^= h[j] >> 15;
        const uint4 *slot = p.jhash + 2u * (h[j] & p.jhash_mask);
        ent[j] = slot[0];
        first[j] = slot[1];
    }
#pragma unroll
    for (int j = 0; j < 2; ++j) {
        const int32_t l = jl[j], r = jr[j];
        bool found = false;
        for (int probe = 0; probe < 8; ++probe) {
            if (probe) {
                const uint4 *slot = p.jhash + 2u * ((h[j] + (uint32_t)probe) & p.jhash_mask);
                ent[j] = slot[0];
                first[j] = slot[1];
            }
            if ((int32_t)ent[j].x == l && (int32_t)ent[j].y == r) { found = true; break; }
            if (ent[j].x == 0x80000000u) break;
        }
        if (found) {
            if ((ent[j].w & SPL_JF_COMPLEX) || (ent[j].w & SPL_JF_COUNT_MASK) > 16u) return false;
            if (!STRANDED && (ent[j].w & SPL_JF_MULTIROW)) return false;
            r_off[j] = ent[j].z;
            r_n[j] = ent[j].w & SPL_JF_COUNT_MASK;
        }
    }
    const uint32_t want = sidx ? 2u : 1u;
    const uint32_t a_b1 = sidx, a_me = (STRANDED ? 2u : 1u) + sidx;
#pragma unroll
    for (int j = 0; j < 2; ++j) {
        for (uint32_t i = 0; i < r_n[j]; ++i) {
            const uint4 rv = i ? p.jrivals[2u * (r_off[j] + i)] : first[j];
            bool earlier = false;
            if (j == 1)
                for (uint32_t i2 = 0; i2 < r_n[0]; ++i2) earlier |= ((i2 ? p.jrivals[2u * (r_off[0] + i2)].y : first[0].y) == rv.y);
            if (earlier) continue;
            const int32_t t = (int32_t)rv.x;
            const uint32_t td = rv.y & 0x3fffffffu;
            const bool strand_ok = !STRANDED || (rv.y >> 30) == want;
            int inside = -1;
            bool cov = false, alpha = false;
            int32_t pu = 0;
#pragma unroll
            for (int a = 0; a < 2; ++a) {
                if (t > jl[a] && t < jr[a]) inside = a;
                if (jl[a] == t) { pu = jr[a]; alpha = true; }
                if (jr[a] == t) { pu = jl[a]; alpha = true; }
            }
#pragma unroll
            for (int b = 0; b < 3; ++b) cov |= (blk_a[b] <= t) && (t + 1 <= blk_b[b]);
            const bool beta1type = !alpha && inside < 0 && cov && strand_ok;
            if (alpha || beta1type) {
                const uint4 rx = p.jrivals[2u * (r_off[j] + i) + 1u];
                for (uint32_t e2 = 0; e2 < rx.z; ++e2) {
                    const int32_t pp = p.part_pos[rx.y + e2];
                    const bool is_end = pp == jl[0] || pp == jr[0] || pp == jl[1] || pp == jr[1];
                    if (is_end && !(alpha && pp == pu)) agg_add(&p.dbl[rx.y + e2], 1);
                }
                if (beta1type) {
                    commit_key<NARR, WIN>(p, lds, wbase, true, (td << 2) | a_b1, -1);
                    commit_key<NARR, WIN>(p, lds, wbase, true, ((td + 1u) << 2) | a_b1, 1);
                    commit_key<NARR, WIN>(p, lds, wbase, true, (td << 2) | a_me, 1);
                    commit_key<NARR, WIN>(p, lds, wbase, true, ((td + 1u) << 2) | a_me, -1);
                }
            } else if (inside >= j && strand_ok) {
                commit_key<NARR, WIN>(p, lds, wbase, true, (td << 2) | a_me, -1);
                commit_key<NARR, WIN>(p, lds, wbase, true, ((td + 1u) << 2) | a_me, 1);
            }
        }
    }
    return true;
}

}


template <bool STRANDED, bool BIG, bool FUSED>
__global__ __launch_bounds__(FUSED ? SPL_BLOCK_FUSED : SPL_BLOCK) __attribute__((amdgpu_waves_per_eu(FUSED ? 5 : 8, 8))) void spl_count_ranges_kernel(const spl_hot_params p)
{
    constexpr int NARR = STRANDED ? 4 : 2;
    constexpr int WIN = STRANDED ? (FUSED ? SPL_WIN_STRANDED_FUSED : SPL_WIN_STRANDED) : SPL_WIN;
    __shared__ int32_t lds_words[NARR * (WIN + 1)];
    spl_lds_i32 *const lds = (spl_lds_i32 *)lds_words;
    constexpr int BLOCK = FUSED ? SPL_BLOCK_FUSED : SPL_BLOCK, NWAVE = BLOCK / 64;
    constexpr int RPT = (int)SPL_TILE_FUSED / SPL_BLOCK_FUSED;
    constexpr uint32_t SEG = FUSED ? SPL_WAVE_READS_FUSED : SPL_WAVE_READS;
    constexpr uint32_t CSHIFT = BIG ? SPL_CHUNK_BIG_SHIFT : SPL_CHUNK_SHIFT;
    constexpr uint32_t TILE = SPL_TILE_FUSED, TILES = FUSED ? (1u << CSHIFT) / TILE : 1u;
    constexpr uint32_t REC_BYTES = FUSED ? (uint32_t)SPL_REC_BYTES_FUSED : 16u, REC_ROOM = REC_BYTES - 64u;
    static_assert(!FUSED || (REC_ROOM >= 16u * TILE && REC_ROOM >= (TILE / 2u) * SPL_REC_OTHER), "a tile's ops, and half a tile's records whatever they are");
    __shared__ uint4 s_rec[REC_BYTES / 16u];
    __shared__ uint16_t s_idx[FUSED ? TILE : 1];
    __shared__ uint32_t s_lay[2 * NWAVE];
    typedef __attribute__((address_space(3))) const char spl_lchar;
    spl_lchar *const lrec = (spl_lchar *)s_rec;
    __shared__ uint16_t s_q[NWAVE * SEG];
    __shared__ uint32_t s_qcnt[NWAVE], s_qbase;
    const uint32_t wave = (uint32_t)__builtin_amdgcn_readfirstlane((int)(threadIdx.x >> 6));
    const uint32_t seg0 = wave * SEG;
    uint32_t lane = (uint32_t)threadIdx.x & 63u;
    uint32_t n_front = 0, n_back = 0, back_done = 0;
    uint32_t fm_mnm = 0, it_mnm = 0;
    auto rank_in = [](unsigned long long m) {
        return (uint32_t)__builtin_amdgcn_mbcnt_hi((uint32_t)(m >> 32), __builtin_amdgcn_mbcnt_lo((uint32_t)m, 0u));
    };
    const uint32_t chunk_slot = my_chunk();
    const uint32_t ordered = chunk_slot < p.n_chunks ? p.chunk_order[chunk_slot] : 0xffffffffu;
    const bool live = ordered != 0xffffffffu;
    const uint32_t chunk = live ? ordered : 0u;
    auto entry_of = [&](uint32_t slot) { return FUSED ? (uint32_t)((__attribute__((address_space(3))) const uint16_t *)s_idx)[slot & 0x3fffu] : slot; };
    auto push_direct = [&](bool want, uint32_t slot, unsigned long long m, uint32_t n) {
        const uint32_t shard = blockIdx.x & 7u;
        uint32_t base = 0;
        if (lane == 0) base = atomicAdd(&p.queue_n[shard * SPL_COUNTER_STRIDE], n);
        base = (uint32_t)__builtin_amdgcn_readfirstlane((int)base);
        if (want) p.queue[(size_t)shard * p.queue_cap + base + rank_in(m)] = (chunk << CSHIFT) | entry_of(slot);
    };
    auto push_front = [&](bool want, uint32_t slot) {
        const unsigned long long m = __ballot(want);
        const uint32_t n = (uint32_t)__popcll(m);
        if (n_front + n_back - back_done + n > SEG) { push_direct(want, slot, m, n); return; }
        if (want) s_q[seg0 + n_front + rank_in(m)] = (uint16_t)entry_of(slot);
        n_front += n;
    };
    auto push_back = [&](bool want, uint32_t slot) {
        const unsigned long long m = __ballot(want);
        const uint32_t n = (uint32_t)__popcll(m);
        if (n_front + n_back + n > SEG) { push_front(want, slot & 0x3fffu); return; }
        if (want) s_q[seg0 + SEG - 1u - n_back - rank_in(m)] = (uint16_t)slot;
        n_back += n;
    };

    int tid = threadIdx.x;
    int32_t wbase = 0;
    ChunkView cv;
    typedef __attribute__((address_space(1))) const uint32_t spl_gdw;
    auto dbk_at = [&](uint32_t s) { return (spl_gdw *)((__attribute__((address_space(1))) const char *)p.dbucket + (size_t)((s << 3) + (s << 2))); };
    auto dbk2 = [&](uint32_t s) { spl_gdw *q = dbk_at(s); spl_dbk e; e.first = q[0]; e.occ = q[1]; e.rival = 0u; return e; };
    auto dbk3 = [&](uint32_t s) { spl_gdw *q = dbk_at(s); spl_dbk e; e.first = q[0]; e.occ = q[1]; e.rival = q[2]; return e; };
    spl_layout_chunk ch;
    uint32_t tile = 0, tile_last = 0;
    uint32_t ob[TILES + 1];
    auto span_of = [&](uint32_t k) {
        const int64_t g0 = ch.lo & ~(int64_t)((1u << CSHIFT) - 1u), hi = ch.lo + ch.n;
        spllay::TileSpan sp;
        sp.cell0 = g0 + (int64_t)k * TILE;
        sp.lo = sp.cell0 > ch.lo ? sp.cell0 : ch.lo;
        sp.hi = sp.cell0 + TILE < hi ? sp.cell0 + TILE : hi;
        uint32_t a = ob[0], b = ob[1];
#pragma unroll
        for (uint32_t q = 1; q < TILES; ++q) { a = k == q ? ob[q] : a; b = k == q ? ob[q + 1] : b; }
        sp.o_lo = a; sp.o_hi = b; sp.o_fetch_hi = ch.o_hi; sp.seg_op0 = ch.seg_op0;
        return sp;
    };
    if constexpr (FUSED) {
        if (!live) return;
        ch = p.cells[chunk];
        const int64_t g0 = ch.lo & ~(int64_t)((1u << CSHIFT) - 1u), hi = ch.lo + ch.n;
        tile = (uint32_t)((ch.lo - g0) >> SPL_TILE_FUSED_SHIFT);
        tile_last = (uint32_t)((hi - 1 - g0) >> SPL_TILE_FUSED_SHIFT);
        const int32_t fp0 = p.src.pos[ch.lo] + ch.shift;
        const spl_dbk e_first = p.dbucket[dbk_slot(p, fp0 - 1)];
#pragma unroll
        for (uint32_t q = 0; q <= TILES; ++q) {
            int64_t i = g0 + (int64_t)q * TILE;
            i = i < ch.lo ? ch.lo : (i > hi ? hi : i);
            ob[q] = q == 0u ? ch.o_lo : (q == TILES ? ch.o_hi : p.src.cig_off[i]);
        }
        for (int j = tid; j < NARR * (WIN + 1); j += BLOCK) lds[j] = 0;
        cv.rec = nullptr;
        cv.wide = (spl_gu32 *)(p.src.cigar + ch.seg_op0);
        cv.shift = ch.shift;
        cv.first_pos = fp0 - ch.shift;
        { uint32_t nv; dbk_resolve(p, fp0 - 1, e_first, wbase, nv); }
    } else {
        cv = chunk_view(p.chunk_meta + chunk);
    }
    typedef uint32_t u32x4_a8 __attribute__((ext_vector_type(4), aligned(8)));
    auto ld_r4 = [&](uint32_t at) {
        if constexpr (FUSED) { const u32x4_a8 v = *(__attribute__((address_space(3))) const u32x4_a8 *)(lrec + at); return make_uint4(v.x, v.y, v.z, v.w); }
        else return ld_g4(cv.rec + (size_t)at);
    };
    auto ld_r2 = [&](uint32_t at) {
        if constexpr (FUSED) { const spl_u32x2 v = *(__attribute__((address_space(3))) const spl_u32x2 *)(lrec + at); return make_uint2(v.x, v.y); }
        else return ld_g2(cv.rec + (size_t)at);
    };
    uint32_t half = 0;
    for (;;) {
    if constexpr (FUSED) {
        lane = spllay::thread_here() & 63u;
        spllay::TileSpan sp = span_of(tile);
        if (half) {
            int64_t mid = sp.cell0 + (int64_t)(TILE / 2u);
            mid = mid < sp.lo ? sp.lo : (mid > sp.hi ? sp.hi : mid);
            const uint32_t o_mid = p.src.cig_off[mid];
            if (half == 1u) { sp.hi = mid; sp.o_hi = o_mid; } else { sp.lo = mid; sp.o_lo = o_mid; }
        }
        uint32_t n[4] = {0, 0, 0, 0};
        bool fits = true;
        if (sp.hi > sp.lo) {
            SimpleInPlace<STRANDED, NARR, WIN, RPT> simple{p, lds, wbase, ch.shift, half == 0u};
            spllay::TileLoads<(int)TILE, RPT> L;
            spllay::tile_issue<(int)TILE, RPT>(p.src, p.src_n_rec, p.src_n_ops, sp, L);
            fits = spllay::tile_finish<(int)TILE, RPT>(p.src, p.src_n_ops, sp, L, (spllay::lay_lds_w32 *)s_rec, (spllay::lay_lds_w32 *)s_lay,
                                                       spllay::RecordsInLds{(spllay::lay_lds_u8 *)s_rec, (spllay::lay_lds_u16 *)s_idx, tile * TILE}, simple, n, REC_ROOM);
        }
        if (!fits) { half = 1u; continue; }
        cv.start[0] = 0; cv.start[1] = 0; cv.start[2] = n[1]; cv.start[3] = n[1] + n[2]; cv.start[4] = n[1] + n[2] + n[3];
        cv.off[0] = 0;
        cv.off[1] = 0;
        cv.off[2] = n[1] * SPL_REC_MNM;
        cv.off[3] = cv.off[2] + n[2] * SPL_REC_M2;
        __syncthreads();
    }
    constexpr uint32_t KS = SPL_K_SIMPLE, KM = SPL_K_MNM;
    uint32_t g_start[SPL_RC_RUNS + 1];
    g_start[0] = 0;
    g_start[1] = (cv.start[1] + 64u * KS - 1u) / (64u * KS);
    g_start[2] = g_start[1] + (cv.start[2] - cv.start[1] + 64u * KM - 1u) / (64u * KM);
    g_start[3] = g_start[2] + ((cv.start[3] - cv.start[2] + 63u) >> 6);
    g_start[4] = g_start[3] + ((cv.start[4] - cv.start[3] + 63u) >> 6);
    const uint32_t g_total = live ? g_start[SPL_RC_RUNS] : 0u;
    typedef uint4 W4;
    W4 cu0 = make_uint4(0, 0, 0, 0), cu1 = make_uint4(0, 0, 0, 0);
    uint32_t cu_i0 = 0;
    auto fetch = [&](uint32_t g) {
        const uint32_t run = (g >= g_start[1] ? 1u : 0u) + (g >= g_start[2] ? 1u : 0u) + (g >= g_start[3] ? 1u : 0u);
        uint32_t gs = 0, n_run = cv.start[1], off = 0, size = SPL_REC_SIMPLE, per = KS;
        if (run == 1u) { gs = g_start[1]; n_run = cv.start[2] - cv.start[1]; off = cv.off[1]; size = SPL_REC_MNM; per = KM; }
        if (run == 2u) { gs = g_start[2]; n_run = cv.start[3] - cv.start[2]; off = cv.off[2]; size = SPL_REC_M2; per = 1u; }
        if (run == 3u) { gs = g_start[3]; n_run = cv.start[4] - cv.start[3]; off = cv.off[3]; size = SPL_REC_OTHER; per = 1u; }
        const uint32_t i0 = (((g - gs) << 6) + lane) * per;

        cu_i0 = i0;
        const uint32_t r = off + (i0 < n_run ? i0 : 0u) * size;
        cu0 = ld_r4(r);
        cu1 = ld_r4(r + 16u);
    };
    if constexpr (!FUSED) { if (wave < g_total) fetch(wave); }
    if constexpr (!FUSED) {
        { const int32_t fp = cv.first_pos + cv.shift; uint32_t nv; const spl_dbk e = p.dbucket[dbk_slot(p, fp - 1)]; dbk_resolve(p, fp - 1, e, wbase, nv); }
        for (int j = tid; j < NARR * (WIN + 1); j += BLOCK) lds[j] = 0;
        __syncthreads();
    }

    {
        uint32_t g = live ? wave : g_start[SPL_RC_RUNS];
        auto fetch_next = [&]() { if constexpr (!FUSED) fetch(g + NWAVE < g_total ? g + NWAVE : g); };
        auto take = [&](uint32_t gs, uint32_t n_run, uint32_t off, uint32_t size, uint32_t per) {
            if constexpr (FUSED) {
                const uint32_t i0 = (((g - gs) << 6) + lane) * per;
                cu_i0 = i0;
                const uint32_t r = off + (i0 < n_run ? i0 : 0u) * size;
                cu0 = ld_r4(r);
                cu1 = ld_r4(r + 16u);
            }
        };
        if constexpr (!FUSED)
        for (; g < g_start[1]; g += NWAVE) {
            take(0u, cv.start[1], 0u, SPL_REC_SIMPLE, KS);
            const uint32_t i0 = cu_i0;
            const W4 r0 = cu0, r1 = cu1;
            const uint32_t n_run = cv.start[1];
            const uint32_t w[8] = {r0.x, r0.y, r0.z, r0.w, r1.x, r1.y, r1.z, r1.w};
            int32_t pos[KS], c1[KS];
            spl_dbk e0[KS], e1[KS];
#pragma unroll
            for (uint32_t j = 0; j < KS; ++j) {
                pos[j] = (int32_t)w[2 * j] + cv.shift;
                c1[j] = pos[j] + (int32_t)(w[2 * j + 1] >> 16);
                e0[j] = dbk2(dbk_slot(p, pos[j] - 1));
                e1[j] = dbk2(dbk_slot(p, c1[j] - 1));
            }
            fetch_next();
#pragma unroll
            for (uint32_t j = 0; j < KS; ++j) {
                int32_t ua, ub; uint32_t nva, nvb;
                dbk_resolve(p, pos[j] - 1, e0[j], ua, nva);
                dbk_resolve(p, c1[j] - 1, e1[j], ub, nvb);
                const int32_t lo = ua + (int32_t)nva;
                const bool emit = i0 + j < n_run && ub > lo;
                uint32_t arr = 0;
                if (STRANDED) arr = (spl_read_strand(w[2 * j + 1] & 0xffffu, p.stranded) == (uint8_t)'-') ? 1u : 0u;
                if (__any(emit)) commit_range<NARR, WIN>(p, lds, wbase, emit, lo, ub, arr);
            }
        }
        for (; g < g_start[2]; g += NWAVE) {
            take(g_start[1], cv.start[2] - cv.start[1], cv.off[1], SPL_REC_MNM, KM);
            const uint32_t i0 = cu_i0;
            const W4 r0 = cu0, r1 = cu1;
            const uint32_t n_run = cv.start[2] - cv.start[1];
            const uint32_t w[8] = {r0.x, r0.y, r0.z, r0.w, r1.x, r1.y, r1.z, r1.w};
            int32_t pos[KM], c0[KM], c1[KM], c2[KM];
            spl_dbk ea[KM], eb[KM], ec[KM], ed[KM];
#pragma unroll
            for (uint32_t j = 0; j < KM; ++j) {
                pos[j] = (int32_t)w[4 * j] + cv.shift;
                c0[j] = pos[j] + (int32_t)(w[4 * j + 1] >> 16); c1[j] = c0[j] + (int32_t)w[4 * j + 2]; c2[j] = c1[j] + (int32_t)w[4 * j + 3];
                ea[j] = dbk2(dbk_slot(p, pos[j] - 1));
                eb[j] = dbk3(dbk_slot(p, c0[j] - 1));
                ec[j] = dbk3(dbk_slot(p, c1[j] - 1));
                ed[j] = dbk2(dbk_slot(p, c2[j] - 1));
            }
            fetch_next();
#pragma unroll
            for (uint32_t j = 0; j < KM; ++j) {
                const bool alive = i0 + j < n_run;
                uint32_t sidx = 0;
                if (STRANDED) sidx = (spl_read_strand(w[4 * j + 1] & 0xffffu, p.stranded) == (uint8_t)'-') ? 1u : 0u;
                const uint32_t a_me = (STRANDED ? 2u : 1u) + sidx;
                int32_t ua, ub; uint32_t nva, nvb, rv1, rv2;
                auto range = [&](uint32_t arr) {
                    const int32_t lo = ua + (int32_t)nva;
                    const bool em = alive && ub > lo;
                    if (__any(em)) commit_range<NARR, WIN>(p, lds, wbase, em, lo, ub, arr);
                    ua = ub; nva = nvb;
                };
                dbk_resolve(p, pos[j] - 1, ea[j], ua, nva);
                dbk_resolve(p, c0[j] - 1, eb[j], ub, nvb, rv1);
                range(sidx);
                dbk_resolve(p, c1[j] - 1, ec[j], ub, nvb, rv2);
                range(a_me);
                dbk_resolve(p, c2[j] - 1, ed[j], ub, nvb);
                range(sidx);
                const bool flagged = alive && ((rv1 | rv2) != 0u);
                if (__any(flagged)) {
                    const uint32_t slot = cv.start[1] + i0 + j;
                    const bool room = KM * it_mnm + j < 32u;
                    push_front(flagged && (p.combine_mode || !room), slot);
                    if (room) fm_mnm |= (flagged && !p.combine_mode ? 1u : 0u) << (KM * it_mnm + j);
                }
            }
            ++it_mnm;
        }
        for (; g < g_start[3]; g += NWAVE) {
            take(g_start[2], cv.start[3] - cv.start[2], cv.off[2], SPL_REC_M2, 1u);
            const uint32_t i0 = cu_i0;
            const W4 r0 = cu0, r1 = cu1;
            const uint32_t slot = cv.start[2] + i0;
            const bool alive = i0 < cv.start[3] - cv.start[2];
            const uint2 ra = make_uint2(r0.x, r0.y), rb = make_uint2(r0.z, r0.w), rc = make_uint2(r1.x, r1.y);
            const int32_t pos = (int32_t)ra.x + cv.shift;
            const uint32_t flag = ra.y & 0xffffu;
            const uint32_t la = ra.y >> 16, d1 = rb.x, lb = rb.y & 0xffffu, lc = rb.y >> 16, d2 = rc.x;
            const int32_t c0 = pos + (int32_t)la, c1 = c0 + (int32_t)d1, c2 = c1 + (int32_t)lb;
            const int32_t c3 = c2 + (int32_t)d2, c4 = c3 + (int32_t)lc;
            uint32_t sidx2 = 0;
            if (STRANDED) sidx2 = (spl_read_strand(flag, p.stranded) == (uint8_t)'-') ? 1u : 0u;
            const uint32_t a_me = (STRANDED ? 2u : 1u) + sidx2;
            const spl_dbk f0 = dbk2(dbk_slot(p, pos - 1)), f1 = dbk3(dbk_slot(p, c0 - 1)), f2 = dbk3(dbk_slot(p, c1 - 1));
            const spl_dbk f3 = dbk3(dbk_slot(p, c2 - 1)), f4 = dbk3(dbk_slot(p, c3 - 1)), f5 = dbk2(dbk_slot(p, c4 - 1));
            fetch_next();
            int32_t ua, ub; uint32_t nva, nvb, rvb;
            uint32_t fl1 = 0, fl2 = 0;
            auto range = [&](uint32_t arr) {
                const int32_t lo = ua + (int32_t)nva;
                const bool em = alive && ub > lo;
                if (__any(em)) commit_range<NARR, WIN>(p, lds, wbase, em, lo, ub, arr);
                ua = ub; nva = nvb;
            };
            dbk_resolve(p, pos - 1, f0, ua, nva);
            dbk_resolve(p, c0 - 1, f1, ub, nvb, rvb);
            range(sidx2);
            fl1 |= rvb;
            dbk_resolve(p, c1 - 1, f2, ub, nvb, rvb);
            range(a_me);
            fl1 |= rvb;
            dbk_resolve(p, c2 - 1, f3, ub, nvb, rvb);
            range(sidx2);
            fl2 |= rvb;
            dbk_resolve(p, c3 - 1, f4, ub, nvb, rvb);
            range(a_me);
            fl2 |= rvb;
            dbk_resolve(p, c4 - 1, f5, ub, nvb);
            range(sidx2);
            const bool flagged = alive && ((fl1 | fl2) != 0u);
            if (__any(flagged)) {
                push_front(flagged && p.combine_mode, slot);
                push_back(flagged && !p.combine_mode, slot | (fl1 << 14) | (fl2 << 15));
            }
        }
        for (; g < g_total; g += NWAVE) {
            take(g_start[3], cv.start[4] - cv.start[3], cv.off[3], SPL_REC_OTHER, 1u);
            const uint32_t i0 = cu_i0;
            const W4 r0 = cu0, r1 = cu1;
            const uint32_t slot = cv.start[3] + i0;
            bool alive = i0 < cv.start[4] - cv.start[3];
            const uint2 ra = make_uint2(r0.x, r0.y), rb = make_uint2(r0.z, r0.w), rc = make_uint2(r1.x, r1.y);
            const int32_t pos = (int32_t)ra.x + cv.shift;
            const uint32_t flag = ra.y & 0xffffu;
            const uint32_t fn = ra.y;
            uint32_t op[SPL_INLINE_OPS] = {rb.x, rb.y, rc.x};
            uint32_t n_ops = rc.y;
            const bool wide = (fn >> SPL_RC_SHIFT) == SPL_RC_WIDE;
            uint32_t o0 = 0;
            if (wide) {
                o0 = op[2];
                op[2] = 0xfu;
            }
            const uint32_t n_inline = wide ? 2u : n_ops;
            bool bad = alive && (int32_t)ra.x < 0;
            const bool literal = alive && !bad && (flag & 4u);
            alive = alive && !bad && !literal;
            uint32_t sidx = 0;
            if (STRANDED) sidx = (spl_read_strand(flag, p.stranded) == (uint8_t)'-') ? 1u : 0u;
            const uint32_t room = (uint32_t)(SPL_COORD_MAX - (pos < 0 ? 0 : pos));
            uint32_t len = 0;
            int32_t cend[SPL_INLINE_OPS];
            uint32_t kind[SPL_INLINE_OPS];
            int32_t pu = 0; uint32_t pnv = 0, prv = 0;
            bool rival = false;
            uint32_t k_next = n_inline;
            bool mine = true;
            for (bool first = true;; first = false) {
#pragma unroll
                for (int k = 0; k < SPL_INLINE_OPS; ++k) {
                    const uint32_t kd = alive ? ((SPL_KIND_TABLE >> (2u * (op[k] & 15u))) & 3u) : 0u;
                    len += kd ? (op[k] >> 4) : 0u;
                    if (kd && len > room) { bad = true; alive = false; }
                    if (first || mine) {
                        cend[k] = pos + (int32_t)len;
                        kind[k] = alive ? kd : 0u;
                    }
                }
                spl_dbk e0 = {0u, 0u, 0u}, ek[SPL_INLINE_OPS];
                if (first) e0 = p.dbucket[dbk_slot(p, pos - 1)];
#pragma unroll
                for (int k = 0; k < SPL_INLINE_OPS; ++k) ek[k] = p.dbucket[dbk_slot(p, cend[k] - 1)];
                if (first) dbk_resolve(p, pos - 1, e0, pu, pnv, prv);
#pragma unroll
                for (int k = 0; k < SPL_INLINE_OPS; ++k) {
                    int32_t u; uint32_t nv, rv;
                    dbk_resolve(p, cend[k] - 1, ek[k], u, nv, rv);
                    const uint32_t kk = (first || mine) ? kind[k] : 0u;
                    const int32_t lo = pu + (int32_t)pnv;
                    const bool emit = kk != 0u && kk != 3u && u > lo;
                    const uint32_t arr = (kk == 2u ? (STRANDED ? 2u : 1u) : 0u) + sidx;
                    rival |= (kk == 2u) & ((prv | rv) != 0u);
                    if (__any(emit)) commit_range<NARR, WIN>(p, lds, wbase, emit, lo, u, arr);
                    if (kk) { pu = u; pnv = nv; prv = rv; }
                }
                const bool more = alive && wide && k_next < n_ops;
                if (!__any(more)) break;
                mine = more;
#pragma unroll
                for (int k = 0; k < SPL_INLINE_OPS; ++k) op[k] = (more && k_next + (uint32_t)k < n_ops) ? cv.wide[o0 + k_next + (uint32_t)k] : 0xfu;
                k_next += (uint32_t)SPL_INLINE_OPS;
            }
            fetch_next();
            if (bad) atomicOr(p.err, SPL_DEV_ERR_RANGE);
            const bool flagged = !literal && alive && rival;
            if (__any(literal || flagged)) push_front(literal || flagged, slot);
        }
        const uint32_t n_m2 = n_back;
        for (uint32_t r0 = 0; r0 < n_m2; r0 += 64u) {
            const uint32_t j = r0 + lane;
            bool undecided = false;
            uint32_t slot = 0;
            if (j < n_m2) {
                const uint32_t entry = s_q[seg0 + SEG - n_back + j];
                slot = entry & 0x3fffu;
                const uint32_t q = cv.off[2] + SPL_REC_M2 * (slot - cv.start[2]);
                const uint2 ra = ld_r2(q), rb = ld_r2(q + 8u), rc = ld_r2(q + 16u);
                const int32_t pos = (int32_t)ra.x + cv.shift;
                uint32_t sidx = 0;
                if (STRANDED) sidx = (spl_read_strand(ra.y & 0xffffu, p.stranded) == (uint8_t)'-') ? 1u : 0u;
                const int32_t c0 = pos + (int32_t)(ra.y >> 16), c1 = c0 + (int32_t)rb.x, c2 = c1 + (int32_t)(rb.y & 0xffffu);
                const int32_t c3 = c2 + (int32_t)rc.x, c4 = c3 + (int32_t)(rb.y >> 16);
                const int32_t jl[2] = {c0 - 1, c2 - 1}, jr[2] = {c1 - 1, c3 - 1};
                const bool jf[2] = {((entry >> 14) & 1u) != 0u, (entry >> 15) != 0u};
                const int32_t blk_a[3] = {pos, c1, c3}, blk_b[3] = {c0 - 1, c2 - 1, c4 - 1};
                undecided = !rivals_inline2<STRANDED, NARR, WIN>(p, lds, wbase, jl, jr, jf, blk_a, blk_b, sidx);
            }
            back_done = r0 + 64u < n_m2 ? r0 + 64u : n_m2;
            if (__any(undecided)) push_front(undecided, slot);
        }
        if (__any(fm_mnm != 0u)) {
            const uint32_t n_run = cv.start[2] - cv.start[1];
            auto fetch_mnm = [&](uint32_t g2) {
                const uint32_t i0 = (((g2 - g_start[1]) << 6) + lane) * KM;
                const uint32_t r = cv.off[1] + (i0 < n_run ? i0 : 0u) * SPL_REC_MNM;
                cu_i0 = i0;
                cu0 = ld_r4(r);
                cu1 = ld_r4(r + 16u);
            };
            uint32_t g2 = g_start[1] + ((wave + NWAVE - (g_start[1] % NWAVE)) % NWAVE), it2 = 0;
            if constexpr (!FUSED) { if (g2 < g_start[2]) fetch_mnm(g2); }
            for (; g2 < g_start[2] && KM * it2 < 32u; g2 += NWAVE, ++it2) {
                const uint32_t bits = (fm_mnm >> (KM * it2)) & ((1u << KM) - 1u);
                if constexpr (FUSED) {
                    if (!__any(bits != 0u)) continue;
                    fetch_mnm(g2);
                }
                const uint32_t i0 = cu_i0;
                const W4 r0 = cu0, r1 = cu1;
                if constexpr (!FUSED) {
                    fetch_mnm(g2 + NWAVE < g_start[2] ? g2 + NWAVE : g2);
                    if (!__any(bits != 0u)) continue;
                }
                const uint32_t w[8] = {r0.x, r0.y, r0.z, r0.w, r1.x, r1.y, r1.z, r1.w};
                bool live[KM], undecided[KM];
                int32_t pos[KM], c0[KM], c1[KM], c2[KM];
                uint32_t h[KM];
                uint4 ent[KM], first[KM];
#pragma unroll
                for (uint32_t k = 0; k < KM; ++k) {
                    live[k] = ((bits >> k) & 1u) != 0u;
                    undecided[k] = false;
                    pos[k] = (int32_t)w[4 * k] + cv.shift;
                    c0[k] = pos[k] + (int32_t)(w[4 * k + 1] >> 16); c1[k] = c0[k] + (int32_t)w[4 * k + 2]; c2[k] = c1[k] + (int32_t)w[4 * k + 3];
                    h[k] = junction_hash(c0[k] - 1, c1[k] - 1);
                    ent[k] = first[k] = make_uint4(0x80000000u, 0u, 0u, 0u);
                    if (live[k]) {
                        const uint4 *hslot = p.jhash + 2u * (h[k] & p.jhash_mask);
                        ent[k] = hslot[0];
                        first[k] = hslot[1];
                    }
                }
#pragma unroll
                for (uint32_t k = 0; k < KM; ++k) {
                    uint32_t sidx = 0;
                    if (STRANDED) sidx = (spl_read_strand(w[4 * k + 1] & 0xffffu, p.stranded) == (uint8_t)'-') ? 1u : 0u;
                    const int32_t blk_a[2] = {pos[k], c1[k]}, blk_b[2] = {c0[k] - 1, c2[k] - 1};
                    if (live[k]) undecided[k] = !rivals_inline_from<STRANDED, NARR, WIN>(p, lds, wbase, c0[k] - 1, c1[k] - 1, h[k], ent[k], first[k], blk_a, blk_b, sidx);
                }
#pragma unroll
                for (uint32_t k = 0; k < KM; ++k)
                    if (__any(undecided[k])) push_front(undecided[k], cv.start[1] + i0 + k);
            }
        }
    }
    if constexpr (!FUSED) break;
    else {
        if (half == 1u) half = 2u;
        else {
            if (tile == tile_last) break;
            ++tile;
            half = 0u;
        }
        fm_mnm = 0; it_mnm = 0; n_back = 0; back_done = 0;
        __syncthreads();
    }
    }
    if constexpr (FUSED) tid = (int)spllay::thread_here();
    if ((tid & 63) == 0) s_qcnt[tid >> 6] = n_front;
    __syncthreads();
    uint32_t q_start[NWAVE + 1];
    q_start[0] = 0;
#pragma unroll
    for (int w = 0; w < NWAVE; ++w) q_start[w + 1] = q_start[w] + s_qcnt[w];
    const uint32_t qn = q_start[NWAVE];
    if (qn) {
        const uint32_t shard = blockIdx.x & 7u;
        if (tid == 0) s_qbase = atomicAdd(&p.queue_n[shard * SPL_COUNTER_STRIDE], qn);
        __syncthreads();
        uint32_t *dst = p.queue + (size_t)shard * p.queue_cap + s_qbase;
        const uint32_t first = chunk << CSHIFT;
        for (uint32_t j = tid; j < qn; j += BLOCK) {
            uint32_t w = 0;
#pragma unroll
            for (int k = 1; k < NWAVE; ++k) w += (j >= q_start[k]) ? 1u : 0u;
            uint32_t base = 0;
#pragma unroll
            for (int k = 0; k < NWAVE; ++k) base = (w == (uint32_t)k) ? q_start[k] : base;
            dst[j] = first | (uint32_t)s_q[w * SEG + (j - base)];
        }
    }
    for (int j = tid; j < NARR * (WIN + 1); j += BLOCK) {
        const int32_t v = lds[j];
        if (v) {
            const int arr = j / (WIN + 1), loc = j - arr * (WIN + 1);
            atomicAdd(&p.diff[(int64_t)arr * p.diff_stride + wbase + loc], v);
        }
    }
}

namespace {

#define SPL_CF_JUNC 4
#define SPL_CF_BLK 5
template <bool STRANDED>
__device__ __forceinline__ bool rivals_table_path(const spl_count_params &p, int32_t pos, uint32_t flag, const uint32_t *ops, uint32_t n_ops)
{
    if (p.combine_mode) return false;
    int32_t blk_a[SPL_CF_BLK], blk_b[SPL_CF_BLK], jl[SPL_CF_JUNC], jr[SPL_CF_JUNC];
    int n_blk = 0, n_j = 0;
    int32_t cur = pos;
    for (uint32_t k = 0; k < n_ops; ++k) {
        const uint32_t op = ops[k];
        const uint32_t code = op & 15u;
        if (!((SPL_PROG_MASK >> code) & 1u)) continue;
        const int32_t d = (int32_t)(op >> 4);
        const int32_t start = cur;
        cur += d;
        if (code == SPL_OP_N) {
            if (n_j == SPL_CF_JUNC) return false;
#pragma unroll
            for (int j = 0; j < SPL_CF_JUNC; ++j) if (j == n_j) { jl[j] = start - 1; jr[j] = cur - 1; }
            ++n_j;
        } else if (code != SPL_OP_D && d >= 2) {
            if (n_blk == SPL_CF_BLK) return false;
#pragma unroll
            for (int j = 0; j < SPL_CF_BLK; ++j) if (j == n_blk) { blk_a[j] = start; blk_b[j] = cur - 1; }
            ++n_blk;
        }
    }
    if (n_j == 0) return true;
    uint32_t r_off[SPL_CF_JUNC], r_n[SPL_CF_JUNC];
    uint4 first_probe[SPL_CF_JUNC];
#pragma unroll
    for (int j = 0; j < SPL_CF_JUNC; ++j) {
        uint32_t h = (uint32_t)jl[j < n_j ? j : 0] * 0x9E3779B1u ^ (uint32_t)jr[j < n_j ? j : 0] * 0x85EBCA77u;
        h ^= h >> 15;
        first_probe[j] = p.jhash[2u * (h & p.jhash_mask)];
    }
#pragma unroll
    for (int j = 0; j < SPL_CF_JUNC; ++j) {
        r_off[j] = 0; r_n[j] = 0;
        if (j >= n_j) continue;
        const int32_t l = jl[j], r = jr[j];
        uint32_t h = (uint32_t)l * 0x9E3779B1u ^ (uint32_t)r * 0x85EBCA77u;
        h ^= h >> 15;
        bool found = false;
        uint4 ent = first_probe[j];
        for (int probe = 0; probe < 8; ++probe) {
            if (probe) ent = p.jhash[2u * ((h + (uint32_t)probe) & p.jhash_mask)];
            if ((int32_t)ent.x == l && (int32_t)ent.y == r) { found = true; break; }
            if (ent.x == 0x80000000u) break;
        }
        if (found) {
            if (ent.w & SPL_JF_COMPLEX) return false;
            if ((ent.w & SPL_JF_COUNT_MASK) > 16u) return false;
            if (!STRANDED && (ent.w & SPL_JF_MULTIROW)) return false;
            r_off[j] = ent.z; r_n[j] = ent.w & SPL_JF_COUNT_MASK;
        }
    }
    const uint32_t want = (spl_read_strand(flag, STRANDED ? p.stranded : 1) == (uint8_t)'-') ? 2u : 1u;
#pragma unroll
    for (int j = 0; j < SPL_CF_JUNC; ++j) {
        for (uint32_t i = 0; i < r_n[j]; ++i) {
            const uint4 rv = p.jrivals[2u * (r_off[j] + i)];
            const uint4 rx = p.jrivals[2u * (r_off[j] + i) + 1u];
            bool earlier = false;
#pragma unroll
            for (int j2 = 0; j2 < SPL_CF_JUNC; ++j2)
                if (j2 < j) for (uint32_t i2 = 0; i2 < r_n[j2]; ++i2) earlier |= (p.jrivals[2u * (r_off[j2] + i2)].y == rv.y);
            if (earlier) continue;
            const int32_t t = (int32_t)rv.x;
            const bool strand_ok = !STRANDED || (rv.y >> 30) == want;
            int inside = -1;
            bool cov = false, alpha = false;
            int32_t pu = 0;
#pragma unroll
            for (int a = 0; a < SPL_CF_JUNC; ++a) {
                if (a >= n_j) break;
                if (t > jl[a] && t < jr[a]) inside = a;
                if (jl[a] == t) { pu = jr[a]; alpha = true; }
                if (jr[a] == t) { pu = jl[a]; alpha = true; }
            }
#pragma unroll
            for (int b = 0; b < SPL_CF_BLK; ++b) cov |= (b < n_blk) && (blk_a[b] <= t) && (t + 1 <= blk_b[b]);
            const bool beta1type = !alpha && inside < 0 && cov && strand_ok;
            if (alpha || beta1type) {
                for (uint32_t e2 = 0; e2 < rx.z; ++e2) {
                    const int32_t pp = p.part_pos[rx.y + e2];
                    bool is_end = false;
#pragma unroll
                    for (int a = 0; a < SPL_CF_JUNC; ++a) is_end |= (a < n_j) && (pp == jl[a] || pp == jr[a]);
                    if (is_end && !(alpha && pp == pu)) agg_add(&p.dbl[rx.y + e2], 1);
                }
                if (beta1type) {
                    agg_add(&p.beta1[rx.x], -1);
                    agg_add(&p.beta2s_reads[rx.x], 1);
                }
            } else if (inside >= j && strand_ok) {
                agg_add(&p.beta2s_reads[rx.x], -1);
            }
        }
    }
    return true;
}

}

template <bool STRANDED>
__global__ __launch_bounds__(64) void spl_count_literal_kernel(const spl_count_params p, const spl_queue_params q)
{
    __shared__ uint32_t s_ops[64][SPL_PACK_SCAN_OPS + 1];
    for (size_t j = (size_t)blockIdx.x * 64 + threadIdx.x; j < q.clear_n16; j += (size_t)gridDim.x * 64) q.clear_region[j] = make_uint4(0, 0, 0, 0);
    for (uint32_t b = gridDim.x - 1u - blockIdx.x; b < (uint32_t)(q.scan_blocks * q.scan_arrays); b += gridDim.x) {
        const uint32_t arr = b / (uint32_t)q.scan_blocks, blk = b - arr * (uint32_t)q.scan_blocks;
        const int32_t *d = q.diff + (int64_t)arr * q.diff_stride;
        const int32_t base = (int32_t)blk * SPL_SCAN_BLOCK;
        int32_t acc = 0;
        for (int j = (int)threadIdx.x; j < SPL_SCAN_BLOCK; j += 64) acc += (base + j < q.n_dpos) ? d[base + j] : 0;
        for (int o = 32; o > 0; o >>= 1) acc += __shfl_down(acc, o);
// ... 429 lines not shown
```

spliser_amd/csrc/spl_layout_tile.h:

```cpp
#ifndef SPL_LAYOUT_TILE_H
#define SPL_LAYOUT_TILE_H
#include <hip/hip_runtime.h>
#include <stdint.h>

#include "spl_pack.h"
#include "spl_devpack.h"

namespace spllay {

typedef uint32_t lay_u32x2 __attribute__((ext_vector_type(2)));
typedef uint32_t lay_u32x4 __attribute__((ext_vector_type(4)));
typedef lay_u32x2 lay_u32x2_a4 __attribute__((aligned(4)));
typedef lay_u32x4 lay_u32x4_a8 __attribute__((aligned(8)));
typedef __attribute__((address_space(3))) uint32_t lay_lds_w32;
typedef __attribute__((address_space(3))) int32_t lay_lds_i32;
typedef __attribute__((address_space(3))) uint8_t lay_lds_u8;
typedef __attribute__((address_space(3))) uint16_t lay_lds_u16;

typedef __attribute__((address_space(3))) const uint32_t lay_lds_u32;
struct StagedOps {
    static constexpr bool padded = true;
    lay_lds_u32 *p;
    __device__ __forceinline__ uint32_t operator()(uint32_t k) const { return p[k]; }
};
__device__ __forceinline__ uint32_t thread_here()
{
    uint32_t t = threadIdx.x;
    asm volatile("" : "+v"(t));
    return t;
}
__device__ __forceinline__ uint32_t row_scan(uint32_t v)
{
    v += (uint32_t)__builtin_amdgcn_update_dpp(0, (int)v, 0x111, 0xf, 0xf, false);
    v += (uint32_t)__builtin_amdgcn_update_dpp(0, (int)v, 0x112, 0xf, 0xf, false);
    v += (uint32_t)__builtin_amdgcn_update_dpp(0, (int)v, 0x114, 0xf, 0xf, false);
    v += (uint32_t)__builtin_amdgcn_update_dpp(0, (int)v, 0x118, 0xf, 0xf, false);
    return v;
}

__device__ __forceinline__ uint32_t wave_scan(uint32_t v)
{
    v += (uint32_t)__builtin_amdgcn_update_dpp(0, (int)v, 0x111, 0xf, 0xf, false);
    v += (uint32_t)__builtin_amdgcn_update_dpp(0, (int)v, 0x112, 0xf, 0xf, false);
    v += (uint32_t)__builtin_amdgcn_update_dpp(0, (int)v, 0x114, 0xf, 0xf, false);
    v += (uint32_t)__builtin_amdgcn_update_dpp(0, (int)v, 0x118, 0xf, 0xf, false);
    v += (uint32_t)__builtin_amdgcn_update_dpp(0, (int)v, 0x142, 0xa, 0xf, false);
    v += (uint32_t)__builtin_amdgcn_update_dpp(0, (int)v, 0x143, 0xc, 0xf, false);
    return v;
}


struct RecordsInMemory {
    static constexpr bool wants_index = false;
    static constexpr bool clip_tier = false;
    uint8_t *rec_base;
    size_t slot_bytes;
    __device__ __forceinline__ uint8_t *rec() const { return rec_base + (size_t)blockIdx.x * slot_bytes; }
    __device__ __forceinline__ void st2(uint32_t d, lay_u32x2 v) const { *(lay_u32x2 *)(rec() + d) = v; }
    __device__ __forceinline__ void st4(uint32_t d, lay_u32x4 v) const { *(lay_u32x4_a8 *)(rec() + d) = v; }
    __device__ __forceinline__ void index(uint32_t, uint32_t) const {}
};
struct RecordsInLds {
    static constexpr bool wants_index = true;
    static constexpr bool clip_tier = true;
    lay_lds_u8 *rec;
    lay_lds_u16 *idx;
    uint32_t base;
    __device__ __forceinline__ void st2(uint32_t d, lay_u32x2 v) const { *(__attribute__((address_space(3))) lay_u32x2 *)(rec + d) = v; }
    __device__ __forceinline__ void st4(uint32_t d, lay_u32x4 v) const { *(__attribute__((address_space(3))) lay_u32x4_a8 *)(rec + d) = v; }
    __device__ __forceinline__ void index(uint32_t q, uint32_t cell_index) const { idx[q] = (uint16_t)(base + cell_index); }
};
struct SimpleAsRecords { static constexpr bool in_place = false; };

struct TileSpan { int64_t cell0, lo, hi; uint32_t o_lo, o_hi, o_fetch_hi, seg_op0; };
template <int C, int R>
struct TileLoads {
    int32_t pos[R];
    uint32_t fw[R / 2];
    uint32_t co[R + 1];
    lay_u32x4 v[R];
};

template <int C, int R>
__device__ __forceinline__ void tile_issue(const spl_devreads &src, int64_t n_rec, int64_t n_ops, const TileSpan &sp, TileLoads<C, R> &L)
{
    static_assert(R == 4 || R == 2, "two or four reads a thread");
    constexpr uint32_t T = C / R, STAGE = 4 * C;
    static_assert(STAGE / (4 * T) == R, "R quads of ops a thread");
    const uint32_t t = thread_here();
    const int64_t g = sp.cell0 + R * (int64_t)t;
#pragma unroll
    for (int j = 0; j < R; ++j) L.pos[j] = 0;
#pragma unroll
    for (int j = 0; j <= R; ++j) L.co[j] = 0;
#pragma unroll
    for (int j = 0; j < R / 2; ++j) L.fw[j] = 0;
    const uint32_t r0 = (uint32_t)R * t, lo_r = (uint32_t)(sp.lo - sp.cell0), hi_r = (uint32_t)(sp.hi - sp.cell0);
    const int64_t left = n_rec - sp.cell0;
    const uint32_t rec_r = left < (int64_t)C ? (uint32_t)left : (uint32_t)C;
    const bool mine = r0 + R > lo_r && r0 < hi_r;
    if (mine) {
        if (r0 + R <= rec_r) {
            if constexpr (R == 4) {
                const lay_u32x4 pv = *(const lay_u32x4 *)(src.pos + g);
                const lay_u32x2 fv = *(const lay_u32x2 *)(src.flag + g);
                const lay_u32x4 cv = *(const lay_u32x4 *)(src.cig_off + g);
                L.co[4] = src.cig_off[g + 4];
                L.pos[0] = (int32_t)pv.x; L.pos[1] = (int32_t)pv.y; L.pos[2] = (int32_t)pv.z; L.pos[3] = (int32_t)pv.w;
                L.fw[0] = fv.x; L.fw[1] = fv.y;
                L.co[0] = cv.x; L.co[1] = cv.y; L.co[2] = cv.z; L.co[3] = cv.w;
            } else {
                const lay_u32x2 pv = *(const lay_u32x2 *)(src.pos + g);
                L.fw[0] = *(const uint32_t *)(src.flag + g);
                const lay_u32x2 cv = *(const lay_u32x2 *)(src.cig_off + g);
                L.co[2] = src.cig_off[g + 2];
                L.pos[0] = (int32_t)pv.x; L.pos[1] = (int32_t)pv.y;
                L.co[0] = cv.x; L.co[1] = cv.y;
            }
        } else {
            uint32_t f[R];
#pragma unroll
            for (int j = 0; j < R; ++j) {
                const int64_t i = g + j;
                f[j] = 0;
                if (i < n_rec) { L.pos[j] = src.pos[i]; f[j] = src.flag[i]; L.co[j] = src.cig_off[i]; L.co[j + 1] = src.cig_off[i + 1]; }
                else L.co[j + 1] = L.co[j];
            }
#pragma unroll
            for (int j = 0; j < R / 2; ++j) L.fw[j] = f[2 * j] | (f[2 * j + 1] << 16);
        }
    }
    const uint64_t ws = sp.o_lo & ~3u;
    const uint64_t o_end = (uint64_t)sp.o_fetch_hi < ws + STAGE ? (uint64_t)sp.o_fetch_hi : ws + STAGE;
#pragma unroll
    for (uint32_t q = 0; q < (uint32_t)R; ++q) {
        const uint64_t at = ws + 4ull * (t + q * T);
        L.v[q] = lay_u32x4{0u, 0u, 0u, 0u};
        if (at < o_end) {
            if (at + 4 <= (uint64_t)n_ops) L.v[q] = *(const lay_u32x4 *)(src.cigar + at);
            else {
                L.v[q].x = src.cigar[at];
                if (at + 1 < (uint64_t)n_ops) L.v[q].y = src.cigar[at + 1];
                if (at + 2 < (uint64_t)n_ops) L.v[q].z = src.cigar[at + 2];
            }
        }
    }
}

template <int C, int R, class Sink, class Simple>
__device__ __forceinline__ bool tile_finish(const spl_devreads &src, int64_t n_ops, const TileSpan &sp, const TileLoads<C, R> &L, lay_lds_w32 *s_ops,
                                            lay_lds_w32 *s_cnt, const Sink sink, Simple &simple, uint32_t (&n)[4], uint32_t room = 0xffffffffu)
{
    constexpr uint32_t T = C / R, NW = T / 64, STAGE = 4 * C;
    static_assert(NW <= 16, "the waves' totals are summed inside one row of lanes");
    constexpr uint32_t PAD = SPL_PACK_SCAN_OPS;
    const uint32_t t = thread_here(), lane = t & 63u, wave = t >> 6;
    const int64_t g = sp.cell0 + R * (int64_t)t;
    const uint32_t r0 = (uint32_t)R * t, lo_r = (uint32_t)(sp.lo - sp.cell0), hi_r = (uint32_t)(sp.hi - sp.cell0);
    const uint32_t o_hi = sp.o_hi, seg_op0 = sp.seg_op0;
    int32_t pos[R];
    uint32_t flag[R], co[R + 1];
#pragma unroll
    for (int j = 0; j < R; ++j) { pos[j] = L.pos[j]; flag[j] = (j & 1) ? L.fw[j / 2] >> 16 : L.fw[j / 2] & 0xffffu; }
#pragma unroll
    for (int j = 0; j <= R; ++j) co[j] = L.co[j];
    auto fill = [&](uint64_t ws) {
        const uint64_t o_end = (uint64_t)o_hi < ws + STAGE ? (uint64_t)o_hi : ws + STAGE;
        lay_u32x4 v[R];
#pragma unroll
        for (uint32_t q = 0; q < (uint32_t)R; ++q) {
            const uint64_t at = ws + 4ull * (t + q * T);
            v[q] = lay_u32x4{0u, 0u, 0u, 0u};
            if (at < o_end) {
                if (at + 4 <= (uint64_t)n_ops) v[q] = *(const lay_u32x4 *)(src.cigar + at);
                else {
                    v[q].x = src.cigar[at];
                    if (at + 1 < (uint64_t)n_ops) v[q].y = src.cigar[at + 1];
                    if (at + 2 < (uint64_t)n_ops) v[q].z = src.cigar[at + 2];
                }
            }
        }
#pragma unroll
        for (uint32_t q = 0; q < (uint32_t)R; ++q) *(__attribute__((address_space(3))) lay_u32x4 *)(s_ops + 4u * (t + q * T)) = v[q];
    };
    uint64_t ws = sp.o_lo & ~3u;
#pragma unroll
    for (uint32_t q = 0; q < (uint32_t)R; ++q) *(__attribute__((address_space(3))) lay_u32x4 *)(s_ops + 4u * (t + q * T)) = L.v[q];
    __syncthreads();

    uint32_t w[R][6];
    uint32_t runs = 0, pend = 0;
#pragma unroll
    for (int j = 0; j < R; ++j) {
        const bool valid = r0 + (uint32_t)j >= lo_r && r0 + (uint32_t)j < hi_r;
        const uint32_t rel0 = co[j] - (uint32_t)ws;
        const bool inside = rel0 + PAD <= STAGE;
        lay_lds_u32 *o = (lay_lds_u32 *)s_ops + (inside ? rel0 : 0u);
        splrec::Rec r;
        bool fast;
        if constexpr (Sink::clip_tier) fast = splrec::classify_plain(pos[j], flag[j], o[0], o[1], o[2], o[3], o[4], co[j + 1] - co[j], r);
        else fast = splrec::classify_fast5(pos[j], flag[j], o[0], o[1], o[2], o[3], o[4], co[j + 1] - co[j], co[j] - seg_op0, r);
        pend |= (valid && !(fast && inside) ? 1u : 0u) << j;
        runs |= (valid ? r.run : (uint32_t)SPL_RC_RUNS) << (3 * j);
#pragma unroll
        for (int q = 0; q < 6; ++q) w[j][q] = r.w[q];
        __builtin_amdgcn_sched_barrier(0);
    }
    if (Sink::clip_tier && __any(pend != 0u)) {
#pragma unroll
        for (int j = 0; j < R; ++j) {
            const uint32_t rel0 = co[j] - (uint32_t)ws;
            const bool inside = rel0 + PAD <= STAGE;
            splrec::Rec r;
            const bool fast = splrec::classify_clipped(pos[j], flag[j], StagedOps{(lay_lds_u32 *)s_ops + (inside ? rel0 : 0u)}, co[j + 1] - co[j], co[j] - seg_op0, r);
            const bool take = ((pend >> j) & 1u) != 0u && fast && inside;
            runs = take ? (runs & ~(7u << (3 * j))) | (r.run << (3 * j)) : runs;
            pend = take ? pend & ~(1u << j) : pend;
#pragma unroll
            for (int q = 0; q < 6; ++q) w[j][q] = take ? r.w[q] : w[j][q];
            __builtin_amdgcn_sched_barrier(0);
        }
    }
    for (;;) {
        if (__any(pend != 0u)) {
#pragma unroll
            for (int j = 0; j < R; ++j) {
                if ((pend >> j) & 1u) {
                    const uint32_t c0 = src.cig_off[g + j], c1 = src.cig_off[g + j + 1], rel0 = c0 - (uint32_t)ws;
                    if (rel0 + PAD <= STAGE) {
                        splrec::Rec r;
                        splrec::classify_lean((int32_t)w[j][0], w[j][1] & 0xffffu, StagedOps{(lay_lds_u32 *)s_ops + rel0}, c1 - c0, c0 - seg_op0, r);
                        runs = (runs & ~(7u << (3 * j))) | (r.run << (3 * j));
                        pend &= ~(1u << j);
#pragma unroll
                        for (int q = 0; q < 6; ++q) w[j][q] = r.w[q];
                    }
                }
                __builtin_amdgcn_sched_barrier(0);
            }
        }
        if (ws + STAGE >= (uint64_t)o_hi + PAD) break;
        ws += STAGE - PAD;
        __syncthreads();
        fill(ws);
        __syncthreads();
    }
    uint32_t c01 = 0, c23 = 0;
    uint32_t run[R];
#pragma unroll
    for (int j = 0; j < R; ++j) {
        run[j] = (runs >> (3 * j)) & 7u;
        if constexpr (Simple::in_place) {
            simple.issue(j, run[j] == SPL_RC_SIMPLE, w[j][0], w[j][1]);
            c01 += run[j] == SPL_RC_MNM ? 0x10000u : 0u;
        } else
        c01 += run[j] == SPL_RC_SIMPLE ? 1u : (run[j] == SPL_RC_MNM ? 0x10000u : 0u);
        c23 += run[j] == SPL_RC_M2 ? 1u : (run[j] == SPL_RC_OTHER ? 0x10000u : 0u);
    }

    const uint32_t i01 = wave_scan(c01), i23 = wave_scan(c23);
    if (lane == 63u) { s_cnt[2u * wave] = i01; s_cnt[2u * wave + 1u] = i23; }
    __syncthreads();
    const uint32_t x = row_scan(lane < NW ? s_cnt[2u * (lane < NW ? lane : 0u)] : 0u), y = row_scan(lane < NW ? s_cnt[2u * (lane < NW ? lane : 0u) + 1u] : 0u);
    const uint32_t wu = (uint32_t)__builtin_amdgcn_readfirstlane((int)wave);
    const uint32_t t01 = (uint32_t)__builtin_amdgcn_readlane((int)x, NW - 1), t23 = (uint32_t)__builtin_amdgcn_readlane((int)y, NW - 1);
    const uint32_t b01 = wu ? (uint32_t)__builtin_amdgcn_readlane((int)x, wu - 1u) : 0u, b23 = wu ? (uint32_t)__builtin_amdgcn_readlane((int)y, wu - 1u) : 0u;
    const uint32_t n0 = t01 & 0xffffu, n1 = t01 >> 16, n2 = t23 & 0xffffu, n3 = t23 >> 16;
    const uint32_t off1 = (n0 * SPL_REC_SIMPLE + 15u) & ~15u, off2 = off1 + n1 * SPL_REC_MNM, off3 = off2 + n2 * SPL_REC_M2;
    n[0] = n0; n[1] = n1; n[2] = n2; n[3] = n3;
    if (off3 + n3 * SPL_REC_OTHER > room) {
        if constexpr (Simple::in_place) {
#pragma unroll
            for (int j = 0; j < R; ++j) simple.commit(j, run[j] == SPL_RC_SIMPLE, w[j][0], w[j][1]);
        }
        return false;
    }
    const uint32_t e01 = b01 + i01 - c01, e23 = b23 + i23 - c23;
    uint32_t at[4] = {(e01 & 0xffffu) * SPL_REC_SIMPLE, off1 + (e01 >> 16) * SPL_REC_MNM, off2 + (e23 & 0xffffu) * SPL_REC_M2, off3 + (e23 >> 16) * SPL_REC_OTHER};
    [[maybe_unused]] uint32_t q_at[3] = {e01 >> 16, n1 + (e23 & 0xffffu), n1 + n2 + (e23 >> 16)};

#pragma unroll
    for (int j = 0; j < R; ++j) {
        const uint32_t r = run[j];
        uint32_t d = r == SPL_RC_MNM ? at[1] : (r == SPL_RC_M2 ? at[2] : at[3]);
        if constexpr (!Simple::in_place) d = r == SPL_RC_SIMPLE ? at[0] : d;
        if (r == SPL_RC_SIMPLE) { if constexpr (!Simple::in_place) sink.st2(d, lay_u32x2{w[j][0], w[j][1]}); }
        else if (r < (uint32_t)SPL_RC_RUNS) {
            sink.st4(d, lay_u32x4{w[j][0], w[j][1], w[j][2], w[j][3]});
            if (r != SPL_RC_MNM) sink.st2(d + 16, lay_u32x2{w[j][4], w[j][5]});
            if constexpr (Sink::wants_index) {
                sink.index(r == SPL_RC_MNM ? q_at[0] : (r == SPL_RC_M2 ? q_at[1] : q_at[2]), (uint32_t)R * t + (uint32_t)j);
                q_at[0] += r == SPL_RC_MNM ? 1u : 0u;
                q_at[1] += r == SPL_RC_M2 ? 1u : 0u;
                q_at[2] += r == SPL_RC_OTHER ? 1u : 0u;
            }
        }
        if constexpr (!Simple::in_place) at[0] += r == SPL_RC_SIMPLE ? SPL_REC_SIMPLE : 0u;
        at[1] += r == SPL_RC_MNM ? SPL_REC_MNM : 0u;
        at[2] += r == SPL_RC_M2 ? SPL_REC_M2 : 0u;
        at[3] += r == SPL_RC_OTHER ? SPL_REC_OTHER : 0u;
    }
    if constexpr (Simple::in_place) {
#pragma unroll
        for (int j = 0; j < R; ++j) simple.commit(j, run[j] == SPL_RC_SIMPLE, w[j][0], w[j][1]);
    }
    return true;
}

template <int C, class Sink>
__device__ __forceinline__ void layout_tile(const spl_devreads &src, int64_t n_rec, int64_t n_ops, const spl_layout_chunk &ch, lay_lds_w32 *s_ops,
                                            lay_lds_w32 *s_cnt, lay_lds_i32 *s_first, const Sink sink, uint32_t (&n)[4])
{
    const TileSpan sp{ch.lo & ~(int64_t)(C - 1), ch.lo, ch.lo + ch.n, ch.o_lo, ch.o_hi, ch.o_hi, ch.seg_op0};
    TileLoads<C, 4> L;
    tile_issue<C, 4>(src, n_rec, n_ops, sp, L);
    const int64_t g = sp.cell0 + 4 * (int64_t)threadIdx.x;
    if (sp.lo >= g && sp.lo < g + 4) {
        const uint32_t e = (uint32_t)(sp.lo - g);
        *s_first = e == 0u ? L.pos[0] : (e == 1u ? L.pos[1] : (e == 2u ? L.pos[2] : L.pos[3]));
    }
    SimpleAsRecords as_records;
    (void)tile_finish<C, 4>(src, n_ops, sp, L, s_ops, s_cnt, sink, as_records, n);
}

}
#endif
```

Measured before the change: 163.2 million.

## Precompute fused chunk descriptors in order kernel and load via scalar constant path

The layout-map kernel now builds a 64-byte per-chunk descriptor holding start, count, shift, first position and the tile CIGAR-offset boundaries. The chunk-order kernel copies these descriptors into cost-sorted slot order. The fused count kernel then reads its chunk parameters with scalar constant-address loads instead of gathering the cell record, pos and cig_off in the prologue. It also reloads kernel params from the kernarg segment, defers the first density-bucket lookup until after staging, and switches tile loads to 32-bit relative offsets. This aims to shorten prologue latency and cut VGPR and 64-bit address work, at the cost of extra descriptor memory and more work in the two setup kernels.

```diff
diff --git a/spliser_amd/csrc/spl_capi.cpp b/spliser_amd/csrc/spl_capi.cpp
--- a/spliser_amd/csrc/spl_capi.cpp
+++ b/spliser_amd/csrc/spl_capi.cpp
@@ -384,6 +384,8 @@
     spl_chunk_meta *meta = nullptr;
     uint32_t *cost = nullptr;
     uint32_t *chunk_order = nullptr;
+    spl_fused_slot *by_chunk = nullptr;
+    spl_fused_slot *slots = nullptr;
     uint32_t *queue = nullptr;
     uint32_t *queue_alt = nullptr;
     uint32_t *queue_total = nullptr;
@@ -2545,13 +2547,13 @@
         lp.src = spl_devreads{(const int32_t *)g.src->pos, (const uint16_t *)g.src->flag, (const uint32_t *)g.src->cig_off, (const uint32_t *)g.src->cigar};
         lp.n_rec = g.src->n_rec; lp.n_ops = g.src->n_ops;
         lp.chunks = g.d_chunks; lp.rec_base = (uint8_t *)g.slab; lp.meta = d->meta;
-        const int rc0 = spl_dev_launch_layout_map(&lp.src, g.d_segs, (uint32_t)g.segs.size(), g.n_chunks, chunk, g.d_chunks, d->cost, c->stream);
+        const int rc0 = spl_dev_launch_layout_map(&lp.src, g.d_segs, (uint32_t)g.segs.size(), g.n_chunks, chunk, g.d_chunks, d->cost, d->by_chunk, c->stream);
         if (rc0) return spl_set_error(SPL_ERR_HIP, "layout map kernel launch: %s", hipGetErrorString((hipError_t)rc0));
         lps.push_back(lp);
     }
     if (d->n_chunks) {
         splprof::Scope prof("spl_chunk_order_kernel", c->stream, 8.0 * (double)d->n_chunks);
-        const int rc = spl_dev_launch_chunk_order(d->cost, d->n_chunks, chunk, d->chunk_order, c->stream);
+        const int rc = spl_dev_launch_chunk_order(d->cost, d->n_chunks, chunk, d->chunk_order, d->by_chunk, d->slots, c->stream);
         if (rc) return spl_set_error(SPL_ERR_HIP, "chunk order kernel launch: %s", hipGetErrorString((hipError_t)rc));
     }
     size_t gi = 0;
@@ -2602,6 +2604,7 @@
     size_t off = 0;
     auto take = [&](size_t bytes) { size_t o = off; off = align_up(off + bytes); return o; };
     const size_t o_meta = take(sizeof(spl_chunk_meta) * std::max<size_t>(n, 1)), o_cost = take(4 * std::max<size_t>(n, 1)), o_order = take(4 * std::max<size_t>(d->n_slots, 1));
+    const size_t o_by_chunk = take(sizeof(spl_fused_slot) * std::max<size_t>(n, 1)), o_slots = take(sizeof(spl_fused_slot) * std::max<size_t>(d->n_slots, 1));
     const size_t o_total = take(4);
     const size_t o_queue = take(4 * 8 * shard_cap), o_queue_alt = take(c->tail ? 4 * 8 * shard_cap : 0);
     hipError_t e = devmem::get((void **)&d->ctl, std::max<size_t>(off, 256), 'c');
@@ -2609,6 +2612,8 @@
     d->meta = (spl_chunk_meta *)(d->ctl + o_meta);
     d->cost = (uint32_t *)(d->ctl + o_cost);
     d->chunk_order = (uint32_t *)(d->ctl + o_order);
+    d->by_chunk = (spl_fused_slot *)(d->ctl + o_by_chunk);
+    d->slots = (spl_fused_slot *)(d->ctl + o_slots);
     d->queue_total = (uint32_t *)(d->ctl + o_total);
     d->queue = (uint32_t *)(d->ctl + o_queue);
     d->queue_alt = c->tail ? (uint32_t *)(d->ctl + o_queue_alt) : d->queue;
@@ -3090,6 +3095,7 @@
     if (dr->fused) {
         const spl_dreads::Group &g = dr->groups[0];
         h.cells = g.d_chunks;
+        h.slots = dr->slots;
         h.src = spl_devreads{(const int32_t *)g.src->pos, (const uint16_t *)g.src->flag, (const uint32_t *)g.src->cig_off, (const uint32_t *)g.src->cigar};
         h.src_n_rec = g.src->n_rec; h.src_n_ops = g.src->n_ops;
     }
diff --git a/spliser_amd/csrc/spl_device.h b/spliser_amd/csrc/spl_device.h
--- a/spliser_amd/csrc/spl_device.h
+++ b/spliser_amd/csrc/spl_device.h
@@ -23,8 +23,6 @@
 #define SPL_WAVE_ITERS 10
 #endif
 #define SPL_WAVE_READS (64 * SPL_WAVE_ITERS)
-#define SPL_TILE_FUSED_SHIFT 10
-#define SPL_TILE_FUSED (1 << SPL_TILE_FUSED_SHIFT)
 #define SPL_BLOCK_FUSED 256
 #define SPL_WAVE_READS_FUSED 512
 #define SPL_REC_BYTES_FUSED 16448
@@ -114,6 +112,7 @@
     uint32_t queue_cap;
     int32_t *err;
     const spl_layout_chunk *cells;
+    const spl_fused_slot *slots;
     spl_devreads src;
     int64_t src_n_rec, src_n_ops;
 };
diff --git a/spliser_amd/csrc/spl_devpack.h b/spliser_amd/csrc/spl_devpack.h
--- a/spliser_amd/csrc/spl_devpack.h
+++ b/spliser_amd/csrc/spl_devpack.h
@@ -31,6 +31,23 @@
     uint32_t flat;
 };
 
+#define SPL_TILE_FUSED_SHIFT 10
+#define SPL_TILE_FUSED (1 << SPL_TILE_FUSED_SHIFT)
+#define SPL_FUSED_TILES_MAX 4
+#define SPL_SLOT_EMPTY 0xffffffffu
+struct alignas(64) spl_fused_slot {
+    int64_t lo;
+    uint32_t chunk;
+    uint32_t n;
+    int32_t shift;
+    uint32_t seg_op0;
+    int32_t pos0;
+    uint32_t unused0;
+    uint32_t ob[SPL_FUSED_TILES_MAX + 1];
+    uint32_t unused1[3];
+};
+static_assert(sizeof(spl_fused_slot) == 64, "one scalar load of sixteen words");
+
 struct spl_layout_params {
     spl_devreads src;
     int64_t n_rec;
@@ -50,9 +67,9 @@
 extern "C" {
 #endif
 int spl_dev_launch_layout_map(const spl_devreads *src, const spl_layout_seg *segs, uint32_t n_segs, uint32_t n_chunks, uint32_t chunk, spl_layout_chunk *chunks, uint32_t *cost,
-                              void *stream);
+                              spl_fused_slot *by_chunk, void *stream);
 int spl_dev_launch_layout(const spl_layout_params *p, uint32_t n_dev_chunks, uint32_t chunk, void *stream, void *ev_start, void *ev_stop);
-int spl_dev_launch_chunk_order(const uint32_t *cost, uint32_t n_chunks, uint32_t chunk, uint32_t *order, void *stream);
+int spl_dev_launch_chunk_order(const uint32_t *cost, uint32_t n_chunks, uint32_t chunk, uint32_t *order, const spl_fused_slot *by_chunk, spl_fused_slot *slots, void *stream);
 #ifdef __cplusplus
 }
 #endif
diff --git a/spliser_amd/csrc/spl_devpack.hip b/spliser_amd/csrc/spl_devpack.hip
--- a/spliser_amd/csrc/spl_devpack.hip
+++ b/spliser_amd/csrc/spl_devpack.hip
@@ -9,7 +9,7 @@
 using namespace spllay;
 
 __global__ __launch_bounds__(256) void spl_layout_map_kernel(const spl_devreads src, const spl_layout_seg *segs, uint32_t n_segs, uint32_t n_chunks, uint32_t chunk,
-                                                             spl_layout_chunk *chunks, uint32_t *cost)
+                                                             spl_layout_chunk *chunks, uint32_t *cost, spl_fused_slot *by_chunk)
 {
     const uint32_t k = blockIdx.x * 256u + threadIdx.x;
     if (k >= n_chunks) return;
@@ -29,6 +29,17 @@
     c.flat = s.chunk0 + (k - s.dev0);
     chunks[k] = c;
     cost[c.flat] = (3u * (c.o_hi - c.o_lo) + c.n) / 2u;
+    spl_fused_slot f;
+    f.lo = c.lo; f.chunk = c.flat; f.n = c.n; f.shift = c.shift; f.seg_op0 = c.seg_op0;
+    f.pos0 = c.n ? src.pos[c.lo] : 0;
+    f.unused0 = 0; f.unused1[0] = f.unused1[1] = f.unused1[2] = 0;
+    const uint32_t tiles = chunk >> SPL_TILE_FUSED_SHIFT;
+    for (uint32_t q = 0; q <= SPL_FUSED_TILES_MAX; ++q) {
+        int64_t i = c0 + (int64_t)q * SPL_TILE_FUSED;
+        i = i < c.lo ? c.lo : (i > hi ? hi : i);
+        f.ob[q] = q == 0u ? c.o_lo : (q >= tiles ? c.o_hi : src.cig_off[i]);
+    }
+    by_chunk[c.flat] = f;
 }
 
 template <int C>
@@ -54,7 +65,8 @@
     }
 }
 
-__global__ __launch_bounds__(1024) void spl_chunk_order_kernel(const uint32_t *cost, uint32_t n, uint32_t per, uint32_t *order)
+__global__ __launch_bounds__(1024) void spl_chunk_order_kernel(const uint32_t *cost, uint32_t n, uint32_t per, uint32_t *order, const spl_fused_slot *by_chunk,
+                                                               spl_fused_slot *slots)
 {
     constexpr uint32_t NB = 4096;
     __shared__ uint32_t s_hist[NB];
@@ -83,18 +95,31 @@
     s_hist[4 * t] = before; s_hist[4 * t + 1] = before + h0; s_hist[4 * t + 2] = before + h0 + h1; s_hist[4 * t + 3] = before + h0 + h1 + h2;
     __syncthreads();
     uint32_t *const mine = order + (size_t)x * per;
+    spl_fused_slot *const mine_slots = slots + (size_t)x * per;
     for (uint32_t e = t; e < per; e += 1024u) {
         const uint32_t j = chunk_of(e);
-        if (j < n) mine[atomicAdd(&s_hist[key_of(cost[j])], 1u)] = j;
+        if (j < n) {
+            const uint32_t dst = atomicAdd(&s_hist[key_of(cost[j])], 1u);
+            mine[dst] = j;
+            const uint4 *from = (const uint4 *)(by_chunk + j);
+            uint4 *to = (uint4 *)(mine_slots + dst);
+            const uint4 a = from[0], b = from[1], c = from[2], d = from[3];
+            to[0] = a; to[1] = b; to[2] = c; to[3] = d;
+        }
     }
-    for (uint32_t s = total + t; s < per; s += 1024u) mine[s] = 0xffffffffu;
+    for (uint32_t s = total + t; s < per; s += 1024u) {
+        mine[s] = 0xffffffffu;
+        uint4 *to = (uint4 *)(mine_slots + s);
+        to[0] = make_uint4(0u, 0u, SPL_SLOT_EMPTY, 0u);
+        to[1] = to[2] = to[3] = make_uint4(0u, 0u, 0u, 0u);
+    }
 }
 
 extern "C" int spl_dev_launch_layout_map(const spl_devreads *src, const spl_layout_seg *segs, uint32_t n_segs, uint32_t n_chunks, uint32_t chunk, spl_layout_chunk *chunks,
-                                         uint32_t *cost, void *stream)
+                                         uint32_t *cost, spl_fused_slot *by_chunk, void *stream)
 {
     if (!n_segs || !n_chunks) return 0;
-    hipLaunchKernelGGL(spl_layout_map_kernel, dim3((n_chunks + 255u) / 256u), dim3(256), 0, (hipStream_t)stream, *src, segs, n_segs, n_chunks, chunk, chunks, cost);
+    hipLaunchKernelGGL(spl_layout_map_kernel, dim3((n_chunks + 255u) / 256u), dim3(256), 0, (hipStream_t)stream, *src, segs, n_segs, n_chunks, chunk, chunks, cost, by_chunk);
     return (int)hipGetLastError();
 }
 
@@ -109,10 +134,11 @@
     return (int)hipGetLastError();
 }
 
-extern "C" int spl_dev_launch_chunk_order(const uint32_t *cost, uint32_t n_chunks, uint32_t chunk, uint32_t *order, void *stream)
+extern "C" int spl_dev_launch_chunk_order(const uint32_t *cost, uint32_t n_chunks, uint32_t chunk, uint32_t *order, const spl_fused_slot *by_chunk, spl_fused_slot *slots,
+                                          void *stream)
 {
     if (!n_chunks) return 0;
     (void)chunk;
-    hipLaunchKernelGGL(spl_chunk_order_kernel, dim3(8), dim3(1024), 0, (hipStream_t)stream, cost, n_chunks, spl_order_per(n_chunks), order);
+    hipLaunchKernelGGL(spl_chunk_order_kernel, dim3(8), dim3(1024), 0, (hipStream_t)stream, cost, n_chunks, spl_order_per(n_chunks), order, by_chunk, slots);
     return (int)hipGetLastError();
 }
diff --git a/spliser_amd/csrc/spl_kernels.hip b/spliser_amd/csrc/spl_kernels.hip
--- a/spliser_amd/csrc/spl_kernels.hip
+++ b/spliser_amd/csrc/spl_kernels.hip
@@ -397,9 +397,25 @@
     static constexpr bool in_place = true;
     const spl_hot_params &p;
     spl_lds_i32 *lds;
-    int32_t wbase, shift;
+    int32_t &wbase;
+    int32_t shift;
     bool active;
+    bool &wbase_pending;
+    const int32_t x_first;
+    uint32_t first_first = 0, first_occ = 0;
     spl_dbk e0[R], e1[R];
+    __device__ __forceinline__ void ask_base()
+    {
+        if (wbase_pending) {
+            typedef __attribute__((address_space(4))) const uint32_t spl_cdw;
+            spl_cdw *const q = (spl_cdw *)((__attribute__((address_space(4))) const char *)(uintptr_t)p.dbucket + (size_t)dbk_slot(p, x_first) * sizeof(spl_dbk));
+            first_first = q[0]; first_occ = q[1];
+        }
+    }
+    __device__ __forceinline__ void staged()
+    {
+        if (wbase_pending) { uint32_t nv; dbk_resolve(p, x_first, spl_dbk{first_first, first_occ, 0u}, wbase, nv); wbase_pending = false; }
+    }
     __device__ __forceinline__ void issue(int j, bool is_simple, uint32_t w0, uint32_t w1)
     {
         if (!active || !__any(is_simple)) return;
@@ -583,8 +599,24 @@
 
 
 template <bool STRANDED, bool BIG, bool FUSED>
-__global__ __launch_bounds__(FUSED ? SPL_BLOCK_FUSED : SPL_BLOCK) __attribute__((amdgpu_waves_per_eu(FUSED ? 5 : 8, 8))) void spl_count_ranges_kernel(const spl_hot_params p)
-{
+__global__ __launch_bounds__(FUSED ? SPL_BLOCK_FUSED : SPL_BLOCK) __attribute__((amdgpu_waves_per_eu(FUSED ? 5 : 8, 8))) void spl_count_ranges_kernel(const spl_hot_params p_in)
+{
+    spl_hot_params p = p_in;
+    [[maybe_unused]] auto params_here = [&]() {
+        if constexpr (FUSED) {
+            typedef __attribute__((address_space(4))) const spl_hot_params spl_cparams;
+            uint64_t a = (uint64_t)(uintptr_t)__builtin_amdgcn_kernarg_segment_ptr();
+            asm volatile("" : "+s"(a));
+            spl_cparams *const c = (spl_cparams *)a;
+            p.n_chunks = c->n_chunks; p.chunk_shift = c->chunk_shift; p.chunk_meta = c->chunk_meta; p.chunk_order = c->chunk_order; p.part_pos = c->part_pos;
+            p.dbucket = c->dbucket; p.n_dbuckets = c->n_dbuckets; p.dbase = c->dbase; p.n_dpos = c->n_dpos; p.stranded = c->stranded;
+            p.diff = c->diff; p.diff_stride = c->diff_stride; p.jhash = c->jhash; p.jhash_mask = c->jhash_mask; p.jrivals = c->jrivals;
+            p.dbl = c->dbl; p.combine_mode = c->combine_mode; p.queue = c->queue; p.queue_n = c->queue_n; p.queue_cap = c->queue_cap; p.err = c->err;
+            p.cells = c->cells; p.slots = c->slots;
+            p.src.pos = c->src.pos; p.src.flag = c->src.flag; p.src.cig_off = c->src.cig_off; p.src.cigar = c->src.cigar;
+            p.src_n_rec = c->src_n_rec; p.src_n_ops = c->src_n_ops;
+        }
+    };
     constexpr int NARR = STRANDED ? 4 : 2;
     constexpr int WIN = STRANDED ? (FUSED ? SPL_WIN_STRANDED_FUSED : SPL_WIN_STRANDED) : SPL_WIN;
     __shared__ int32_t lds_words[NARR * (WIN + 1)];
@@ -612,7 +644,16 @@
         return (uint32_t)__builtin_amdgcn_mbcnt_hi((uint32_t)(m >> 32), __builtin_amdgcn_mbcnt_lo((uint32_t)m, 0u));
     };
     const uint32_t chunk_slot = my_chunk();
-    const uint32_t ordered = chunk_slot < p.n_chunks ? p.chunk_order[chunk_slot] : 0xffffffffu;
+    typedef __attribute__((address_space(4))) const spl_fused_slot spl_cslot;
+    auto slot_here = [&]() {
+        uint64_t a = (uint64_t)(uintptr_t)(p.slots + chunk_slot);
+        asm volatile("" : "+s"(a));
+        return (spl_cslot *)a;
+    };
+    uint32_t ordered = 0xffffffffu;
+    if (chunk_slot < p.n_chunks) {
+        if constexpr (FUSED) ordered = slot_here()->chunk; else ordered = p.chunk_order[chunk_slot];
+    }
     const bool live = ordered != 0xffffffffu;
     const uint32_t chunk = live ? ordered : 0u;
     auto entry_of = [&](uint32_t slot) { return FUSED ? (uint32_t)((__attribute__((address_space(3))) const uint16_t *)s_idx)[slot & 0x3fffu] : slot; };
@@ -645,44 +686,38 @@
     auto dbk_at = [&](uint32_t s) { return (spl_gdw *)((__attribute__((address_space(1))) const char *)p.dbucket + (size_t)((s << 3) + (s << 2))); };
     auto dbk2 = [&](uint32_t s) { spl_gdw *q = dbk_at(s); spl_dbk e; e.first = q[0]; e.occ = q[1]; e.rival = 0u; return e; };
     auto dbk3 = [&](uint32_t s) { spl_gdw *q = dbk_at(s); spl_dbk e; e.first = q[0]; e.occ = q[1]; e.rival = q[2]; return e; };
-    spl_layout_chunk ch;
     uint32_t tile = 0, tile_last = 0;
-    uint32_t ob[TILES + 1];
+    static_assert(!FUSED || TILES <= SPL_FUSED_TILES_MAX, "the descriptor's boundaries");
     auto span_of = [&](uint32_t k) {
-        const int64_t g0 = ch.lo & ~(int64_t)((1u << CSHIFT) - 1u), hi = ch.lo + ch.n;
+        spl_cslot *const d = slot_here();
+        const uint32_t first_r = (uint32_t)d->lo & ((1u << CSHIFT) - 1u), end_r = first_r + d->n;
+        const uint32_t t0 = k * TILE;
         spllay::TileSpan sp;
-        sp.cell0 = g0 + (int64_t)k * TILE;
-        sp.lo = sp.cell0 > ch.lo ? sp.cell0 : ch.lo;
-        sp.hi = sp.cell0 + TILE < hi ? sp.cell0 + TILE : hi;
-        uint32_t a = ob[0], b = ob[1];
-#pragma unroll
-        for (uint32_t q = 1; q < TILES; ++q) { a = k == q ? ob[q] : a; b = k == q ? ob[q + 1] : b; }
-        sp.o_lo = a; sp.o_hi = b; sp.o_fetch_hi = ch.o_hi; sp.seg_op0 = ch.seg_op0;
+        sp.cell0 = (d->lo & ~(int64_t)((1u << CSHIFT) - 1u)) + (int64_t)t0;
+        sp.lo_r = first_r > t0 ? first_r - t0 : 0u;
+        sp.hi_r = end_r - t0 < TILE ? end_r - t0 : TILE;
+        sp.o_lo = d->ob[k]; sp.o_hi = d->ob[k + 1u]; sp.o_fetch_hi = d->ob[TILES]; sp.seg_op0 = d->seg_op0;
         return sp;
     };
+    bool wbase_pending = FUSED;
     if constexpr (FUSED) {
         if (!live) return;
-        ch = p.cells[chunk];
-        const int64_t g0 = ch.lo & ~(int64_t)((1u << CSHIFT) - 1u), hi = ch.lo + ch.n;
-        tile = (uint32_t)((ch.lo - g0) >> SPL_TILE_FUSED_SHIFT);
-        tile_last = (uint32_t)((hi - 1 - g0) >> SPL_TILE_FUSED_SHIFT);
-        const int32_t fp0 = p.src.pos[ch.lo] + ch.shift;
-        const spl_dbk e_first = p.dbucket[dbk_slot(p, fp0 - 1)];
-#pragma unroll
-        for (uint32_t q = 0; q <= TILES; ++q) {
-            int64_t i = g0 + (int64_t)q * TILE;
-            i = i < ch.lo ? ch.lo : (i > hi ? hi : i);
-            ob[q] = q == 0u ? ch.o_lo : (q == TILES ? ch.o_hi : p.src.cig_off[i]);
-        }
+        spl_cslot *const d = slot_here();
+        const uint32_t first_r = (uint32_t)d->lo & ((1u << CSHIFT) - 1u);
+        tile = first_r >> SPL_TILE_FUSED_SHIFT;
+        tile_last = (first_r + d->n - 1u) >> SPL_TILE_FUSED_SHIFT;
+        cv.rec = nullptr;
+        cv.wide = nullptr;
+        cv.shift = d->shift;
+        cv.first_pos = 0;
         for (int j = tid; j < NARR * (WIN + 1); j += BLOCK) lds[j] = 0;
-        cv.rec = nullptr;
-        cv.wide = (spl_gu32 *)(p.src.cigar + ch.seg_op0);
-        cv.shift = ch.shift;
-        cv.first_pos = fp0 - ch.shift;
-        { uint32_t nv; dbk_resolve(p, fp0 - 1, e_first, wbase, nv); }
     } else {
         cv = chunk_view(p.chunk_meta + chunk);
     }
+    auto wide_ops = [&]() {
+        if constexpr (FUSED) return (spl_gu32 *)(p.src.cigar + slot_here()->seg_op0);
+        else return cv.wide;
+    };
     typedef uint32_t u32x4_a8 __attribute__((ext_vector_type(4), aligned(8)));
     auto ld_r4 = [&](uint32_t at) {
         if constexpr (FUSED) { const u32x4_a8 v = *(__attribute__((address_space(3))) const u32x4_a8 *)(lrec + at); return make_uint4(v.x, v.y, v.z, v.w); }
@@ -695,20 +730,22 @@
     uint32_t half = 0;
     for (;;) {
     if constexpr (FUSED) {
+        params_here();
         lane = spllay::thread_here() & 63u;
         spllay::TileSpan sp = span_of(tile);
         if (half) {
-            int64_t mid = sp.cell0 + (int64_t)(TILE / 2u);
-            mid = mid < sp.lo ? sp.lo : (mid > sp.hi ? sp.hi : mid);
-            const uint32_t o_mid = p.src.cig_off[mid];
-            if (half == 1u) { sp.hi = mid; sp.o_hi = o_mid; } else { sp.lo = mid; sp.o_lo = o_mid; }
+            uint32_t mid = TILE / 2u;
+            mid = mid < sp.lo_r ? sp.lo_r : (mid > sp.hi_r ? sp.hi_r : mid);
+            const uint32_t o_mid = p.src.cig_off[sp.cell0 + (int64_t)mid];
+            if (half == 1u) { sp.hi_r = mid; sp.o_hi = o_mid; } else { sp.lo_r = mid; sp.o_lo = o_mid; }
         }
         uint32_t n[4] = {0, 0, 0, 0};
         bool fits = true;
-        if (sp.hi > sp.lo) {
-            SimpleInPlace<STRANDED, NARR, WIN, RPT> simple{p, lds, wbase, ch.shift, half == 0u};
+        if (sp.hi_r > sp.lo_r) {
+            SimpleInPlace<STRANDED, NARR, WIN, RPT> simple{p, lds, wbase, cv.shift, half == 0u, wbase_pending, wbase_pending ? slot_here()->pos0 + cv.shift - 1 : 0};
             spllay::TileLoads<(int)TILE, RPT> L;
             spllay::tile_issue<(int)TILE, RPT>(p.src, p.src_n_rec, p.src_n_ops, sp, L);
+            simple.ask_base();
             fits = spllay::tile_finish<(int)TILE, RPT>(p.src, p.src_n_ops, sp, L, (spllay::lay_lds_w32 *)s_rec, (spllay::lay_lds_w32 *)s_lay,
                                                        spllay::RecordsInLds{(spllay::lay_lds_u8 *)s_rec, (spllay::lay_lds_u16 *)s_idx, tile * TILE}, simple, n, REC_ROOM);
         }
@@ -719,6 +756,7 @@
         cv.off[2] = n[1] * SPL_REC_MNM;
         cv.off[3] = cv.off[2] + n[2] * SPL_REC_M2;
         __syncthreads();
+        params_here();
     }
     constexpr uint32_t KS = SPL_K_SIMPLE, KM = SPL_K_MNM;
     uint32_t g_start[SPL_RC_RUNS + 1];
@@ -840,6 +878,7 @@
             }
             ++it_mnm;
         }
+        params_here();
         for (; g < g_start[3]; g += NWAVE) {
             take(g_start[2], cv.start[3] - cv.start[2], cv.off[2], SPL_REC_M2, 1u);
             const uint32_t i0 = cu_i0;
@@ -887,6 +926,7 @@
                 push_back(flagged && !p.combine_mode, slot | (fl1 << 14) | (fl2 << 15));
             }
         }
+        params_here();
         for (; g < g_total; g += NWAVE) {
             take(g_start[3], cv.start[4] - cv.start[3], cv.off[3], SPL_REC_OTHER, 1u);
             const uint32_t i0 = cu_i0;
@@ -951,7 +991,7 @@
                 if (!__any(more)) break;
                 mine = more;
 #pragma unroll
-                for (int k = 0; k < SPL_INLINE_OPS; ++k) op[k] = (more && k_next + (uint32_t)k < n_ops) ? cv.wide[o0 + k_next + (uint32_t)k] : 0xfu;
+                for (int k = 0; k < SPL_INLINE_OPS; ++k) op[k] = (more && k_next + (uint32_t)k < n_ops) ? wide_ops()[o0 + k_next + (uint32_t)k] : 0xfu;
                 k_next += (uint32_t)SPL_INLINE_OPS;
             }
             fetch_next();
@@ -959,6 +999,7 @@
             const bool flagged = !literal && alive && rival;
             if (__any(literal || flagged)) push_front(literal || flagged, slot);
         }
+        params_here();
         const uint32_t n_m2 = n_back;
         for (uint32_t r0 = 0; r0 < n_m2; r0 += 64u) {
             const uint32_t j = r0 + lane;
@@ -982,6 +1023,7 @@
             back_done = r0 + 64u < n_m2 ? r0 + 64u : n_m2;
             if (__any(undecided)) push_front(undecided, slot);
         }
+        params_here();
         if (__any(fm_mnm != 0u)) {
             const uint32_t n_run = cv.start[2] - cv.start[1];
             auto fetch_mnm = [&](uint32_t g2) {
@@ -1049,6 +1091,7 @@
         __syncthreads();
     }
     }
+    params_here();
     if constexpr (FUSED) tid = (int)spllay::thread_here();
     if ((tid & 63) == 0) s_qcnt[tid >> 6] = n_front;
     __syncthreads();
diff --git a/spliser_amd/csrc/spl_layout_tile.h b/spliser_amd/csrc/spl_layout_tile.h
--- a/spliser_amd/csrc/spl_layout_tile.h
+++ b/spliser_amd/csrc/spl_layout_tile.h
@@ -72,7 +72,21 @@
 };
 struct SimpleAsRecords { static constexpr bool in_place = false; };
 
-struct TileSpan { int64_t cell0, lo, hi; uint32_t o_lo, o_hi, o_fetch_hi, seg_op0; };
+struct TileSpan { int64_t cell0; uint32_t lo_r, hi_r; uint32_t o_lo, o_hi, o_fetch_hi, seg_op0; };
+typedef __attribute__((address_space(1))) const char lay_gchar;
+template <class V>
+__device__ __forceinline__ V ld_at(lay_gchar *base, uint32_t byte_off) { return *(__attribute__((address_space(1))) const V *)(base + (size_t)byte_off); }
+__device__ __forceinline__ lay_u32x4 ld_ops_quad(lay_gchar *win, uint32_t rel, uint32_t n_win)
+{
+    lay_u32x4 v = lay_u32x4{0u, 0u, 0u, 0u};
+    if (rel + 4u <= n_win) v = ld_at<lay_u32x4>(win, 4u * rel);
+    else {
+        v.x = ld_at<uint32_t>(win, 4u * rel);
+        if (rel + 1u < n_win) v.y = ld_at<uint32_t>(win, 4u * rel + 4u);
+        if (rel + 2u < n_win) v.z = ld_at<uint32_t>(win, 4u * rel + 8u);
+    }
+    return v;
+}
 template <int C, int R>
 struct TileLoads {
     int32_t pos[R];
@@ -88,32 +102,43 @@
     constexpr uint32_t T = C / R, STAGE = 4 * C;
     static_assert(STAGE / (4 * T) == R, "R quads of ops a thread");
     const uint32_t t = thread_here();
-    const int64_t g = sp.cell0 + R * (int64_t)t;
+    lay_gchar *const pos_c = (lay_gchar *)(src.pos + sp.cell0), *const flag_c = (lay_gchar *)(src.flag + sp.cell0), *const co_c = (lay_gchar *)(src.cig_off + sp.cell0);
 #pragma unroll
     for (int j = 0; j < R; ++j) L.pos[j] = 0;
 #pragma unroll
     for (int j = 0; j <= R; ++j) L.co[j] = 0;
 #pragma unroll
     for (int j = 0; j < R / 2; ++j) L.fw[j] = 0;
-    const uint32_t r0 = (uint32_t)R * t, lo_r = (uint32_t)(sp.lo - sp.cell0), hi_r = (uint32_t)(sp.hi - sp.cell0);
+    const uint32_t ws = sp.o_lo & ~3u;
+    lay_gchar *const win = (lay_gchar *)(src.cigar + ws);
+    const uint32_t end_r = sp.o_fetch_hi - ws < STAGE ? sp.o_fetch_hi - ws : STAGE;
+    const int64_t ops_left = n_ops - (int64_t)ws;
+    const uint32_t n_win = ops_left < (int64_t)(STAGE + 4u) ? (uint32_t)ops_left : STAGE + 4u;
+#pragma unroll
+    for (uint32_t q = 0; q < (uint32_t)R; ++q) {
+        const uint32_t rel = 4u * (t + q * T);
+        L.v[q] = lay_u32x4{0u, 0u, 0u, 0u};
+        if (rel < end_r) L.v[q] = ld_ops_quad(win, rel, n_win);
+    }
+    const uint32_t r0 = (uint32_t)R * t, lo_r = sp.lo_r, hi_r = sp.hi_r;
     const int64_t left = n_rec - sp.cell0;
     const uint32_t rec_r = left < (int64_t)C ? (uint32_t)left : (uint32_t)C;
     const bool mine = r0 + R > lo_r && r0 < hi_r;
     if (mine) {
         if (r0 + R <= rec_r) {
             if constexpr (R == 4) {
-                const lay_u32x4 pv = *(const lay_u32x4 *)(src.pos + g);
-                const lay_u32x2 fv = *(const lay_u32x2 *)(src.flag + g);
-                const lay_u32x4 cv = *(const lay_u32x4 *)(src.cig_off + g);
-                L.co[4] = src.cig_off[g + 4];
+                const lay_u32x4 pv = ld_at<lay_u32x4>(pos_c, 4u * r0);
+                const lay_u32x2 fv = ld_at<lay_u32x2>(flag_c, 2u * r0);
+                const lay_u32x4 cv = ld_at<lay_u32x4>(co_c, 4u * r0);
+                L.co[4] = ld_at<uint32_t>(co_c, 4u * r0 + 16u);
                 L.pos[0] = (int32_t)pv.x; L.pos[1] = (int32_t)pv.y; L.pos[2] = (int32_t)pv.z; L.pos[3] = (int32_t)pv.w;
                 L.fw[0] = fv.x; L.fw[1] = fv.y;
                 L.co[0] = cv.x; L.co[1] = cv.y; L.co[2] = cv.z; L.co[3] = cv.w;
             } else {
-                const lay_u32x2 pv = *(const lay_u32x2 *)(src.pos + g);
-                L.fw[0] = *(const uint32_t *)(src.flag + g);
-                const lay_u32x2 cv = *(const lay_u32x2 *)(src.cig_off + g);
-                L.co[2] = src.cig_off[g + 2];
+                const lay_u32x2 pv = ld_at<lay_u32x2>(pos_c, 4u * r0);
+                L.fw[0] = ld_at<uint32_t>(flag_c, 2u * r0);
+                const lay_u32x2 cv = ld_at<lay_u32x2>(co_c, 4u * r0);
+                L.co[2] = ld_at<uint32_t>(co_c, 4u * r0 + 8u);
                 L.pos[0] = (int32_t)pv.x; L.pos[1] = (int32_t)pv.y;
                 L.co[0] = cv.x; L.co[1] = cv.y;
             }
@@ -121,28 +146,13 @@
             uint32_t f[R];
 #pragma unroll
             for (int j = 0; j < R; ++j) {
-                const int64_t i = g + j;
+                const uint32_t i = r0 + (uint32_t)j;
                 f[j] = 0;
-                if (i < n_rec) { L.pos[j] = src.pos[i]; f[j] = src.flag[i]; L.co[j] = src.cig_off[i]; L.co[j + 1] = src.cig_off[i + 1]; }
+                if (i < rec_r) { L.pos[j] = ld_at<int32_t>(pos_c, 4u * i); f[j] = ld_at<uint16_t>(flag_c, 2u * i); L.co[j] = ld_at<uint32_t>(co_c, 4u * i); L.co[j + 1] = ld_at<uint32_t>(co_c, 4u * i + 4u); }
                 else L.co[j + 1] = L.co[j];
             }
 #pragma unroll
             for (int j = 0; j < R / 2; ++j) L.fw[j] = f[2 * j] | (f[2 * j + 1] << 16);
-        }
-    }
-    const uint64_t ws = sp.o_lo & ~3u;
-    const uint64_t o_end = (uint64_t)sp.o_fetch_hi < ws + STAGE ? (uint64_t)sp.o_fetch_hi : ws + STAGE;
-#pragma unroll
-    for (uint32_t q = 0; q < (uint32_t)R; ++q) {
-        const uint64_t at = ws + 4ull * (t + q * T);
-        L.v[q] = lay_u32x4{0u, 0u, 0u, 0u};
-        if (at < o_end) {
-            if (at + 4 <= (uint64_t)n_ops) L.v[q] = *(const lay_u32x4 *)(src.cigar + at);
-            else {
-                L.v[q].x = src.cigar[at];
-                if (at + 1 < (uint64_t)n_ops) L.v[q].y = src.cigar[at + 1];
-                if (at + 2 < (uint64_t)n_ops) L.v[q].z = src.cigar[at + 2];
-            }
         }
     }
 }
@@ -155,8 +165,7 @@
     static_assert(NW <= 16, "the waves' totals are summed inside one row of lanes");
     constexpr uint32_t PAD = SPL_PACK_SCAN_OPS;
     const uint32_t t = thread_here(), lane = t & 63u, wave = t >> 6;
-    const int64_t g = sp.cell0 + R * (int64_t)t;
-    const uint32_t r0 = (uint32_t)R * t, lo_r = (uint32_t)(sp.lo - sp.cell0), hi_r = (uint32_t)(sp.hi - sp.cell0);
+    const uint32_t r0 = (uint32_t)R * t, lo_r = sp.lo_r, hi_r = sp.hi_r;
     const uint32_t o_hi = sp.o_hi, seg_op0 = sp.seg_op0;
     int32_t pos[R];
     uint32_t flag[R], co[R + 1];
@@ -164,36 +173,33 @@
     for (int j = 0; j < R; ++j) { pos[j] = L.pos[j]; flag[j] = (j & 1) ? L.fw[j / 2] >> 16 : L.fw[j / 2] & 0xffffu; }
 #pragma unroll
     for (int j = 0; j <= R; ++j) co[j] = L.co[j];
-    auto fill = [&](uint64_t ws) {
-        const uint64_t o_end = (uint64_t)o_hi < ws + STAGE ? (uint64_t)o_hi : ws + STAGE;
+    auto fill = [&](uint32_t ws) {
+        lay_gchar *const win = (lay_gchar *)(src.cigar + ws);
+        const uint32_t end_r = o_hi - ws < STAGE ? o_hi - ws : STAGE;
+        const int64_t ops_left = n_ops - (int64_t)ws;
+        const uint32_t n_win = ops_left < (int64_t)(STAGE + 4u) ? (uint32_t)ops_left : STAGE + 4u;
         lay_u32x4 v[R];
 #pragma unroll
         for (uint32_t q = 0; q < (uint32_t)R; ++q) {
-            const uint64_t at = ws + 4ull * (t + q * T);
+            const uint32_t rel = 4u * (t + q * T);
             v[q] = lay_u32x4{0u, 0u, 0u, 0u};
-            if (at < o_end) {
-                if (at + 4 <= (uint64_t)n_ops) v[q] = *(const lay_u32x4 *)(src.cigar + at);
-                else {
-                    v[q].x = src.cigar[at];
-                    if (at + 1 < (uint64_t)n_ops) v[q].y = src.cigar[at + 1];
-                    if (at + 2 < (uint64_t)n_ops) v[q].z = src.cigar[at + 2];
-                }
-            }
+            if (rel < end_r) v[q] = ld_ops_quad(win, rel, n_win);
         }
 #pragma unroll
         for (uint32_t q = 0; q < (uint32_t)R; ++q) *(__attribute__((address_space(3))) lay_u32x4 *)(s_ops + 4u * (t + q * T)) = v[q];
     };
-    uint64_t ws = sp.o_lo & ~3u;
+    uint32_t ws = sp.o_lo & ~3u;
 #pragma unroll
     for (uint32_t q = 0; q < (uint32_t)R; ++q) *(__attribute__((address_space(3))) lay_u32x4 *)(s_ops + 4u * (t + q * T)) = L.v[q];
     __syncthreads();
+    if constexpr (Simple::in_place) simple.staged();
 
     uint32_t w[R][6];
     uint32_t runs = 0, pend = 0;
 #pragma unroll
     for (int j = 0; j < R; ++j) {
         const bool valid = r0 + (uint32_t)j >= lo_r && r0 + (uint32_t)j < hi_r;
-        const uint32_t rel0 = co[j] - (uint32_t)ws;
+        const uint32_t rel0 = co[j] - ws;
         const bool inside = rel0 + PAD <= STAGE;
         lay_lds_u32 *o = (lay_lds_u32 *)s_ops + (inside ? rel0 : 0u);
         splrec::Rec r;
@@ -209,7 +215,7 @@
     if (Sink::clip_tier && __any(pend != 0u)) {
 #pragma unroll
         for (int j = 0; j < R; ++j) {
-            const uint32_t rel0 = co[j] - (uint32_t)ws;
+            const uint32_t rel0 = co[j] - ws;
             const bool inside = rel0 + PAD <= STAGE;
             splrec::Rec r;
             const bool fast = splrec::classify_clipped(pos[j], flag[j], StagedOps{(lay_lds_u32 *)s_ops + (inside ? rel0 : 0u)}, co[j + 1] - co[j], co[j] - seg_op0, r);
@@ -226,7 +232,8 @@
 #pragma unroll
             for (int j = 0; j < R; ++j) {
                 if ((pend >> j) & 1u) {
-                    const uint32_t c0 = src.cig_off[g + j], c1 = src.cig_off[g + j + 1], rel0 = c0 - (uint32_t)ws;
+                    lay_gchar *const co_c = (lay_gchar *)(src.cig_off + sp.cell0);
+                    const uint32_t c0 = ld_at<uint32_t>(co_c, 4u * (r0 + (uint32_t)j)), c1 = ld_at<uint32_t>(co_c, 4u * (r0 + (uint32_t)j) + 4u), rel0 = c0 - ws;
                     if (rel0 + PAD <= STAGE) {
                         splrec::Rec r;
                         splrec::classify_lean((int32_t)w[j][0], w[j][1] & 0xffffu, StagedOps{(lay_lds_u32 *)s_ops + rel0}, c1 - c0, c0 - seg_op0, r);
@@ -239,7 +246,7 @@
                 __builtin_amdgcn_sched_barrier(0);
             }
         }
-        if (ws + STAGE >= (uint64_t)o_hi + PAD) break;
+        if (o_hi - ws + PAD <= STAGE) break;
         ws += STAGE - PAD;
         __syncthreads();
         fill(ws);
@@ -311,12 +318,13 @@
 __device__ __forceinline__ void layout_tile(const spl_devreads &src, int64_t n_rec, int64_t n_ops, const spl_layout_chunk &ch, lay_lds_w32 *s_ops,
                                             lay_lds_w32 *s_cnt, lay_lds_i32 *s_first, const Sink sink, uint32_t (&n)[4])
 {
-    const TileSpan sp{ch.lo & ~(int64_t)(C - 1), ch.lo, ch.lo + ch.n, ch.o_lo, ch.o_hi, ch.o_hi, ch.seg_op0};
+    const int64_t cell0 = ch.lo & ~(int64_t)(C - 1);
+    const TileSpan sp{cell0, (uint32_t)(ch.lo - cell0), (uint32_t)(ch.lo - cell0) + ch.n, ch.o_lo, ch.o_hi, ch.o_hi, ch.seg_op0};
     TileLoads<C, 4> L;
     tile_issue<C, 4>(src, n_rec, n_ops, sp, L);
-    const int64_t g = sp.cell0 + 4 * (int64_t)threadIdx.x;
-    if (sp.lo >= g && sp.lo < g + 4) {
-        const uint32_t e = (uint32_t)(sp.lo - g);
+    const uint32_t r0 = 4u * threadIdx.x;
+    if (sp.lo_r >= r0 && sp.lo_r < r0 + 4u) {
+        const uint32_t e = sp.lo_r - r0;
         *s_first = e == 0u ? L.pos[0] : (e == 1u ? L.pos[1] : (e == 2u ? L.pos[2] : L.pos[3]));
     }
     SimpleAsRecords as_records;
```

Result: faster. 169.9 million (median of 6 runs) (+4.1%).
